# yinyunie/Pose2Room

Hardware: AMD Instinct MI355X
Metric: P2RNet train-step samples/sec (T=1024,J=53,bs=32) (higher is better)
Workload: dtype f32; 1 GPU; P2RNet full train step, bs=32/GPU, T=1024, J=53, seeds=512, proposals=128 (BASELINE configs[2]); input=P2RNet_dataloader over SyntheticPoseDataset, global_batch=32, frames=1024, parallelism=dp1

## Files before the change

### pose2room_amd/csrc/p2r_common.h

```cpp
#pragma once
#include <hip/hip_runtime.h>
#include <stdint.h>

#include "../../include/p2r_hip.h"

#pragma clang fp contract(off)

#define P2R_WAVE 64

#define P2R_LAUNCH_CHECK()                      \
  do {                                          \
    hipError_t e__ = hipGetLastError();         \
    if (e__ != hipSuccess) return (int)e__;     \
  } while (0)

static inline hipStream_t p2r_stream(void *s) { return (hipStream_t)s; }

static inline int p2r_ref_opt_n_threads(int work_size) {
  if (work_size <= 0) return 1;
  const int pow_2 = (int)(__builtin_log((double)work_size) / __builtin_log(2.0));
  int t = 1 << pow_2;
  if (t > 512) t = 512;
  if (t < 1) t = 1;
  return t;
}

static inline int p2r_cdiv(long long a, long long b) { return (int)((a + b - 1) / b); }

#define P2R_MAX_DEVICES 64
template <typename K>
static inline hipError_t p2r_allow_big_lds(K kernel, unsigned char (&done)[P2R_MAX_DEVICES], int bytes = 160 * 1024) {
  int dev = 0;
  hipError_t e = hipGetDevice(&dev);
  if (e != hipSuccess) return e;
  if (dev >= 0 && dev < P2R_MAX_DEVICES && done[dev]) return hipSuccess;
  e = hipFuncSetAttribute((const void *)kernel, hipFuncAttributeMaxDynamicSharedMemorySize, bytes);
  if (e == hipSuccess && dev >= 0 && dev < P2R_MAX_DEVICES) done[dev] = 1;
  return e;
}

template <auto KERNEL, typename... Args>
static inline int p2r_launch_big_lds(int blocks, int threads, size_t lds, void *stream, Args... args) {
  static unsigned char lds_ok[P2R_MAX_DEVICES];
  hipError_t e = p2r_allow_big_lds(KERNEL, lds_ok);
  if (e != hipSuccess) return (int)e;
  hipLaunchKernelGGL(KERNEL, dim3(blocks), dim3(threads), lds, p2r_stream(stream), args...);
  P2R_LAUNCH_CHECK();
  return P2R_OK;
}

__device__ __forceinline__ float p2r_sqdist(float ax, float ay, float az,
                                            float bx, float by, float bz) {
  const float dx = ax - bx, dy = ay - by, dz = az - bz;
  return dx * dx + dy * dy + dz * dz;
}

__device__ __forceinline__ float p2r_row16_sum(float v) {
  v += __int_as_float(__builtin_amdgcn_update_dpp(0, __float_as_int(v), 0xB1, 0xf, 0xf, false));
  v += __int_as_float(__builtin_amdgcn_update_dpp(0, __float_as_int(v), 0x4E, 0xf, 0xf, false));
  v += __int_as_float(__builtin_amdgcn_update_dpp(0, __float_as_int(v), 0x141, 0xf, 0xf, false));
  v += __int_as_float(__builtin_amdgcn_update_dpp(0, __float_as_int(v), 0x140, 0xf, 0xf, false));
  return v;
}
```

### pose2room_amd/csrc/pw_layers.hip

```cpp
#include "pw_mma.h"

namespace {

constexpr int PW_COLS = 64;
constexpr int PW_KMAX = 560;

struct PwJobs { p2r_pw_job j[P2R_PW_MAX_JOBS]; };

__global__ __launch_bounds__(256) void pw_gemm_kernel(PwJobs jobs, int L, int colblocks) {
  extern __shared__ float tile[];
  const p2r_pw_job &J = jobs.j[blockIdx.x / colblocks];
  const int cb = blockIdx.x % colblocks;
  const int col0 = cb * PW_COLS;
  const int b = col0 / L, l0 = col0 - b * L;
  const int tid = threadIdx.x, lane = tid & 63, wave = tid >> 6;
  const int g = lane >> 4, r = lane & 15;
  const int K = J.k, kpad = (K + 15) & ~15, rows = J.rows;

  if (!J.x_nlc) {
    const int c4 = tid & 15;
    const size_t base = (size_t)b * J.x_ctot * L + l0 + 4 * c4;
    for (int row = tid >> 4; row < kpad; row += 16) {
      float4 v = make_float4(0.f, 0.f, 0.f, 0.f);
      if (row < K) {
        v = *reinterpret_cast<const float4 *>(J.x + base + (size_t)row * L);
        if (J.tr_mode == 1) {
          const float s = J.tr[row], t = J.tr[J.tr_ld + row];
          v.x = fmaxf(v.x * s + t, 0.f); v.y = fmaxf(v.y * s + t, 0.f);
          v.z = fmaxf(v.z * s + t, 0.f); v.w = fmaxf(v.w * s + t, 0.f);
        } else if (J.tr_mode == 2) {
          const float4 z = *reinterpret_cast<const float4 *>(J.x2 + base + (size_t)row * L);
          const float a = J.tr[row], bq = J.tr[J.tr_ld + row], c = J.tr[2 * J.tr_ld + row];
          v.x = a * v.x + bq * z.x + c; v.y = a * v.y + bq * z.y + c;
          v.z = a * v.z + bq * z.z + c; v.w = a * v.w + bq * z.w + c;
        }
      }
      *reinterpret_cast<float4 *>(tile + row * PW_RS + 4 * c4) = v;
    }
  } else if ((K & 3) != 0 || (J.x_ctot & 3) != 0) {
    const int col = tid & 63;
    const size_t base = ((size_t)b * L + l0 + col) * J.x_ctot;
    for (int row = tid >> 6; row < kpad; row += 4) {
      float v = 0.f;
      if (row < K) {
        v = J.x[base + row];
        if (J.tr_mode == 1) v = fmaxf(v * J.tr[row] + J.tr[J.tr_ld + row], 0.f);
        else if (J.tr_mode == 2) v = J.tr[row] * v + J.tr[J.tr_ld + row] * J.x2[base + row] + J.tr[2 * J.tr_ld + row];
      }
      tile[row * PW_RS + col] = v;
    }
  } else {
    const int col = tid & 63;
    const size_t base = ((size_t)b * L + l0 + col) * J.x_ctot;
    for (int c4 = tid >> 6; c4 < (kpad >> 2); c4 += 4) {
      const int row = 4 * c4;
      float v[4] = {0.f, 0.f, 0.f, 0.f};
      if (row < K) {
        const float4 u = *reinterpret_cast<const float4 *>(J.x + base + row);
        v[0] = u.x; v[1] = u.y; v[2] = u.z; v[3] = u.w;
        if (J.tr_mode == 1) {
#pragma unroll
          for (int e = 0; e < 4; ++e) v[e] = fmaxf(v[e] * J.tr[row + e] + J.tr[J.tr_ld + row + e], 0.f);
        } else if (J.tr_mode == 2) {
          const float4 z4 = *reinterpret_cast<const float4 *>(J.x2 + base + row);
          const float z[4] = {z4.x, z4.y, z4.z, z4.w};
#pragma unroll
          for (int e = 0; e < 4; ++e)
            v[e] = J.tr[row + e] * v[e] + J.tr[J.tr_ld + row + e] * z[e] + J.tr[2 * J.tr_ld + row + e];
        }
      }
#pragma unroll
      for (int e = 0; e < 4; ++e) tile[(row + e) * PW_RS + col] = v[e];
    }
  }
  __syncthreads();

  const int mtiles = (rows + 15) >> 4;
  const int per = (mtiles + 3) >> 2;
  const int lo = wave * per, hi = min(lo + per, mtiles);
  const int nch = kpad >> 4;
  const bool nlc_vec = J.out_nlc && (rows & 3) == 0 && (J.out_ctot & 3) == 0 && (((size_t)J.out) & 15) == 0;
  for (int mt0 = lo; mt0 < hi; mt0 += 4) {
    const int nmt = min(4, hi - mt0);
    floatx4v acc[4][4];
#pragma unroll
    for (int m = 0; m < 4; ++m)
#pragma unroll
      for (int n = 0; n < 4; ++n) acc[m][n] = floatx4v{0.f, 0.f, 0.f, 0.f};
    int rowm[4];
#pragma unroll
    for (int m = 0; m < 4; ++m) rowm[m] = min(16 * (mt0 + m) + r, rows - 1);
    if (J.w_t) pw_product<true>(J.w, tile, K, rows, nch, nmt, rowm, g, r, acc);
    else pw_product<false>(J.w, tile, K, rows, nch, nmt, rowm, g, r, acc);

#pragma unroll
    for (int m = 0; m < 4; ++m) {
      if (m >= nmt) continue;
      const int row0 = 16 * (mt0 + m) + 4 * g;
      float v[4][4];
#pragma unroll
      for (int q = 0; q < 4; ++q) {
        const int row = row0 + q;
        const bool ok = row < rows;
        if (J.epilogue == 0) {
          const float bb = (J.bias && ok) ? J.bias[row] : 0.f;
#pragma unroll
          for (int n = 0; n < 4; ++n) v[q][n] = acc[m][n][q] + bb;
          if (J.stats) {
            float s = (v[q][0] + v[q][1]) + (v[q][2] + v[q][3]);
            s = p2r_row16_sum(s);
            const float mean = s * (1.f / 64.f);
            float d2 = 0.f;
#pragma unroll
            for (int n = 0; n < 4; ++n) { const float d = v[q][n] - mean; d2 += d * d; }
            d2 = p2r_row16_sum(d2);
            if (r == 0 && ok) {
              float *e = J.stats + ((size_t)cb * rows + row) * 3;
              e[0] = 64.f; e[1] = mean; e[2] = d2;
            }
          }
        } else {
          float sc = 0.f, sh = 0.f, mean = 0.f, invstd = 0.f;
          if (ok) {
            mean = J.mfin[row]; invstd = J.mfin[J.mfin_ld + row];
            sc = J.mfin[2 * J.mfin_ld + row]; sh = J.mfin[3 * J.mfin_ld + row];
          }
          float s1 = 0.f, s2 = 0.f;
#pragma unroll
          for (int n = 0; n < 4; ++n) {
            float z = 0.f;
            if (ok) z = J.mz[((size_t)b * J.mz_ctot + row) * L + l0 + 16 * n + r];
            const float gv = (z * sc + sh > 0.f) ? acc[m][n][q] : 0.f;
            v[q][n] = gv;
            s1 += gv;
            s2 += gv * ((z - mean) * invstd);
          }
          if (J.stats) {
            s1 = p2r_row16_sum(s1);
            s2 = p2r_row16_sum(s2);
            if (r == 0 && ok) {
              float *e = J.stats + ((size_t)cb * rows + row) * 2;
              e[0] = s1; e[1] = s2;
            }
          }
        }
      }
      if (!J.out_nlc) {
#pragma unroll
        for (int q = 0; q < 4; ++q)
          if (row0 + q < rows) {
            float *o = J.out + ((size_t)b * J.out_ctot + row0 + q) * L + l0 + r;
#pragma unroll
            for (int n = 0; n < 4; ++n) o[16 * n] = v[q][n];
          }
      } else {
#pragma unroll
        for (int n = 0; n < 4; ++n) {
          float *o = J.out + ((size_t)b * L + l0 + 16 * n + r) * J.out_ctot + row0;
          if (nlc_vec) {
            if (row0 < rows) *reinterpret_cast<float4 *>(o) = make_float4(v[0][n], v[1][n], v[2][n], v[3][n]);
          } else {
#pragma unroll
            for (int q = 0; q < 4; ++q)
              if (row0 + q < rows) o[q] = v[q][n];
          }
        }
      }
    }
  }
}

struct PwWJobs { p2r_pw_wjob j[P2R_PW_MAX_JOBS]; int blk0[P2R_PW_MAX_JOBS + 1]; };
constexpr int PWW_RS = 68;

__device__ __forceinline__ void pww_fetch(const float *__restrict__ p, int ctot, int nlc, int L, int b, int l0, int row_lo,
                                          int nrows, int tid, float4 (&v)[4]) {
#pragma unroll
  for (int i = 0; i < 4; ++i) {
    v[i] = make_float4(0.f, 0.f, 0.f, 0.f);
    if (!nlc) {
      const int row = row_lo + (tid >> 4) + 16 * i;
      if (row < nrows) v[i] = *reinterpret_cast<const float4 *>(p + ((size_t)b * ctot + row) * L + l0 + 4 * (tid & 15));
    } else {
      const int row = row_lo + 4 * ((tid >> 6) + 4 * i);
      const float *q = p + ((size_t)b * L + l0 + (tid & 63)) * ctot;
      if (((nrows | ctot) & 3) == 0) {
        if (row < nrows) v[i] = *reinterpret_cast<const float4 *>(q + row);
      } else {
        if (row + 0 < nrows) v[i].x = q[row + 0];
        if (row + 1 < nrows) v[i].y = q[row + 1];
        if (row + 2 < nrows) v[i].z = q[row + 2];
        if (row + 3 < nrows) v[i].w = q[row + 3];
      }
    }
  }
}

__global__ __launch_bounds__(256) void pw_wgrad_kernel(PwWJobs jobs, int L, int chunks) {
  __shared__ float as[64 * PWW_RS], bs[64 * PWW_RS];
  int ji = 0;
#pragma unroll
  for (int i = 1; i < P2R_PW_MAX_JOBS; ++i)
    if ((int)blockIdx.x >= jobs.blk0[i]) ji = i;
  const p2r_pw_wjob &J = jobs.j[ji];
  const int local = blockIdx.x - jobs.blk0[ji];
  const int rows = J.rows, K = J.k;
  const int tiles_m = (rows + 63) >> 6, tiles_n = (K + 63) >> 6;
  const int sp = local / (tiles_m * tiles_n), t = local % (tiles_m * tiles_n);
  const int tm = t / tiles_n, tn = t % tiles_n;
  const int cps = (chunks + J.split - 1) / J.split;
  const int c_lo = sp * cps, c_hi = min(c_lo + cps, chunks);
  const int tid = threadIdx.x, lane = tid & 63, wave = tid >> 6;
  const int g = lane >> 4, r = lane & 15;
  const int row_a = 64 * tm, row_b = 64 * tn;

  floatx4v acc[4];
#pragma unroll
  for (int mt = 0; mt < 4; ++mt) acc[mt] = floatx4v{0.f, 0.f, 0.f, 0.f};
  float bsum = 0.f;
  const bool want_b = J.db_part != nullptr && tn == 0;

  float4 ra[4], ra2[4], rb[4];
#pragma unroll
  for (int i = 0; i < 4; ++i) ra2[i] = make_float4(0.f, 0.f, 0.f, 0.f);
  if (c_lo < c_hi) {
    const int col0 = c_lo * 64, b = col0 / L, l0 = col0 - b * L;
    pww_fetch(J.x, J.x_ctot, J.x_nlc, L, b, l0, row_a, rows, tid, ra);
    if (J.tr_mode == 2) pww_fetch(J.x2, J.x_ctot, J.x_nlc, L, b, l0, row_a, rows, tid, ra2);
    pww_fetch(J.y, J.y_ctot, J.y_nlc, L, b, l0, row_b, K, tid, rb);
  }
  for (int c = c_lo; c < c_hi; ++c) {
    __syncthreads();
#pragma unroll
    for (int i = 0; i < 4; ++i) {
      const float va[4] = {ra[i].x, ra[i].y, ra[i].z, ra[i].w};
      const float vz[4] = {ra2[i].x, ra2[i].y, ra2[i].z, ra2[i].w};
      const float vb[4] = {rb[i].x, rb[i].y, rb[i].z, rb[i].w};
      if (!J.x_nlc) {
        const int lr = (tid >> 4) + 16 * i, row = row_a + lr;
        float o[4] = {0.f, 0.f, 0.f, 0.f};
        if (row < rows) {
          if (J.tr_mode == 2) {
            const float a = J.tr[row], bq = J.tr[J.tr_ld + row], cc = J.tr[2 * J.tr_ld + row];
#pragma unroll
            for (int e = 0; e < 4; ++e) o[e] = a * va[e] + bq * vz[e] + cc;
          } else {
#pragma unroll
            for (int e = 0; e < 4; ++e) o[e] = va[e];
          }
        }
        *reinterpret_cast<float4 *>(as + lr * PWW_RS + 4 * (tid & 15)) = make_float4(o[0], o[1], o[2], o[3]);
      } else {
#pragma unroll
        for (int e = 0; e < 4; ++e) {
          const int lr = 4 * ((tid >> 6) + 4 * i) + e, row = row_a + lr;
          float v = 0.f;
          if (row < rows) v = J.tr_mode == 2 ? J.tr[row] * va[e] + J.tr[J.tr_ld + row] * vz[e] + J.tr[2 * J.tr_ld + row] : va[e];
          as[lr * PWW_RS + (tid & 63)] = v;
        }
      }
      if (!J.y_nlc) {
        const int lr = (tid >> 4) + 16 * i, row = row_b + lr;
        float o[4] = {0.f, 0.f, 0.f, 0.f};
        if (row < K) {
          if (J.ytr) {
            const float sc = J.ytr[row], sh = J.ytr[J.ytr_ld + row];
#pragma unroll
            for (int e = 0; e < 4; ++e) o[e] = fmaxf(vb[e] * sc + sh, 0.f);
          } else {
#pragma unroll
            for (int e = 0; e < 4; ++e) o[e] = vb[e];
          }
        }
        *reinterpret_cast<float4 *>(bs + lr * PWW_RS + 4 * (tid & 15)) = make_float4(o[0], o[1], o[2], o[3]);
      } else {
#pragma unroll
        for (int e = 0; e < 4; ++e) {
          const int lr = 4 * ((tid >> 6) + 4 * i) + e, row = row_b + lr;
          float v = 0.f;
          if (row < K) v = J.ytr ? fmaxf(vb[e] * J.ytr[row] + J.ytr[J.ytr_ld + row], 0.f) : vb[e];
          bs[lr * PWW_RS + (tid & 63)] = v;
        }
      }
    }
    __syncthreads();
    if (c + 1 < c_hi) {
      const int col0 = (c + 1) * 64, b = col0 / L, l0 = col0 - b * L;
      pww_fetch(J.x, J.x_ctot, J.x_nlc, L, b, l0, row_a, rows, tid, ra);
      if (J.tr_mode == 2) pww_fetch(J.x2, J.x_ctot, J.x_nlc, L, b, l0, row_a, rows, tid, ra2);
      pww_fetch(J.y, J.y_ctot, J.y_nlc, L, b, l0, row_b, K, tid, rb);
    }
#pragma unroll 4
    for (int k = 0; k < 64; k += 4) {
      const float bv = bs[(16 * wave + r) * PWW_RS + k + g];
#pragma unroll
      for (int mt = 0; mt < 4; ++mt)
        acc[mt] = __builtin_amdgcn_mfma_f32_16x16x4f32(as[(16 * mt + r) * PWW_RS + k + g], bv, acc[mt], 0, 0, 0);
    }
    if (want_b) {
      const float *rowp = as + (tid >> 2) * PWW_RS + 16 * (tid & 3);
      float s = 0.f;
#pragma unroll
      for (int i = 0; i < 16; ++i) s += rowp[i];
      bsum += s;
    }
  }
  float *outp = J.dw_part + (size_t)sp * rows * K;
#pragma unroll
  for (int mt = 0; mt < 4; ++mt)
#pragma unroll
    for (int q = 0; q < 4; ++q) {
      const int row = row_a + 16 * mt + 4 * g + q, col = row_b + 16 * wave + r;
      if (row < rows && col < K) outp[(size_t)row * K + col] = acc[mt][q];
    }
  if (want_b) {
    bsum += __shfl_xor(bsum, 1);
    bsum += __shfl_xor(bsum, 2);
    const int row = row_a + (tid >> 2);
    if ((tid & 3) == 0 && row < rows) J.db_part[(size_t)sp * rows + row] = bsum;
  }
}

struct PwBnJobs { p2r_pw_bnjob j[P2R_PW_MAX_JOBS]; int ch0[P2R_PW_MAX_JOBS + 1]; };
struct PwBnbJobs { p2r_pw_bnbjob j[P2R_PW_MAX_JOBS]; int ch0[P2R_PW_MAX_JOBS + 1]; };

__device__ __forceinline__ double wave_sum(double v) {
#pragma unroll
  for (int off = 32; off >= 1; off >>= 1) v += __shfl_xor(v, off);
  return v;
}

__global__ __launch_bounds__(64) void pw_bn_finalize_kernel(PwBnJobs jobs) {
  int ji = 0;
#pragma unroll
  for (int i = 1; i < P2R_PW_MAX_JOBS; ++i)
    if ((int)blockIdx.x >= jobs.ch0[i]) ji = i;
  const p2r_pw_bnjob &J = jobs.j[ji];
  const int c = blockIdx.x - jobs.ch0[ji];
  const int lane = threadIdx.x;
  double mean, var, count = 0.0;
  if (J.part) {
    double n = 0.0, s = 0.0;
    for (int p = lane; p < J.P; p += 64) {
      const float *e = J.part + ((size_t)p * J.C + c) * 3;
      n += (double)e[0]; s += (double)e[0] * (double)e[1];
    }
    n = wave_sum(n); s = wave_sum(s);
    mean = s / n;
    double m2 = 0.0;
    for (int p = lane; p < J.P; p += 64) {
      const float *e = J.part + ((size_t)p * J.C + c) * 3;
      const double d = (double)e[1] - mean;
      m2 += (double)e[2] + (double)e[0] * d * d;
    }
    m2 = wave_sum(m2);
    var = m2 / n;
    if (var < 0.0) var = 0.0;
    count = n;
  } else {
    mean = (double)J.running_mean[c];
    var = (double)J.running_var[c];
  }
  if (lane == 0) {
    const float mean_f = (float)mean, invstd_f = (float)(1.0 / sqrt(var + J.eps));
    const float scale = J.gamma[c] * invstd_f;
    J.fin[c] = mean_f;
    J.fin[J.fin_ld + c] = invstd_f;
    J.fin[2 * J.fin_ld + c] = scale;
    J.fin[3 * J.fin_ld + c] = J.beta[c] - mean_f * scale;
    if (J.part && J.momentum >= 0.0) {
      const float mom = (float)J.momentum;
      const double unbiased = var * (count / (count - 1.0 > 1.0 ? count - 1.0 : 1.0));
      J.running_mean[c] = J.running_mean[c] * (1.f - mom) + mom * mean_f;
      J.running_var[c] = J.running_var[c] * (1.f - mom) + mom * (float)unbiased;
      if (c == 0 && J.num_batches_tracked) *J.num_batches_tracked += 1;
    }
  }
}

__global__ __launch_bounds__(64) void pw_bn_bwd_finalize_kernel(PwBnbJobs jobs) {
  int ji = 0;
#pragma unroll
  for (int i = 1; i < P2R_PW_MAX_JOBS; ++i)
    if ((int)blockIdx.x >= jobs.ch0[i]) ji = i;
  const p2r_pw_bnbjob &J = jobs.j[ji];
  const int c = blockIdx.x - jobs.ch0[ji];
  const int lane = threadIdx.x;
  double s = 0.0, q = 0.0;
  for (int p = lane; p < J.P; p += 64) {
    const float *e = J.part + ((size_t)p * J.C + c) * 2;
    s += (double)e[0]; q += (double)e[1];
  }
  s = wave_sum(s); q = wave_sum(q);
  if (lane == 0) {
    if (J.dbeta) J.dbeta[c] = (float)s;
    if (J.dgamma) J.dgamma[c] = (float)q;
    const float mean = J.fin[c], invstd = J.fin[J.fin_ld + c], scale = J.fin[2 * J.fin_ld + c];
    if (J.train) {
      const float m1 = (float)(s / J.M), m2 = (float)(q / J.M);
      J.coef[c] = scale;
      J.coef[J.coef_ld + c] = -scale * invstd * m2;
      J.coef[2 * J.coef_ld + c] = -scale * m1 + scale * invstd * m2 * mean;
    } else {
      J.coef[c] = scale;
      J.coef[J.coef_ld + c] = 0.f;
      J.coef[2 * J.coef_ld + c] = 0.f;
    }
  }
}

struct PwRJobs { p2r_pw_rjob j[P2R_PW_MAX_RJOBS]; int blk0[P2R_PW_MAX_RJOBS + 1]; };

__global__ __launch_bounds__(256) void pw_reduce_kernel(PwRJobs jobs, int njobs) {
  int ji = 0;
  for (int i = 1; i < njobs; ++i)
    if ((int)blockIdx.x >= jobs.blk0[i]) ji = i;
  const p2r_pw_rjob &J = jobs.j[ji];
  const int i = (blockIdx.x - jobs.blk0[ji]) * 256 + threadIdx.x;
  if (i >= J.M) return;
  float a0 = 0.f, a1 = 0.f, a2 = 0.f, a3 = 0.f;
  int p = 0;
  for (; p + 4 <= J.P; p += 4) {
    a0 += J.in[(size_t)(p + 0) * J.M + i];
    a1 += J.in[(size_t)(p + 1) * J.M + i];
    a2 += J.in[(size_t)(p + 2) * J.M + i];
    a3 += J.in[(size_t)(p + 3) * J.M + i];
  }
  for (; p < J.P; ++p) a0 += J.in[(size_t)p * J.M + i];
  J.out[i] = (a0 + a1) + (a2 + a3);
}

constexpr int MIX_DMAX = 4;
struct MixHeads { p2r_mix_head h[P2R_MIX_MAX_HEADS]; };

template <typename T>
__device__ __forceinline__ void mix_forward_body(const p2r_mix_head &H, int cols, int G, int L, int ctot, double *red) {
  const int tid = threadIdx.x, c = tid & 15, s = tid >> 4;
  const int col = blockIdx.x * 16 + c;
  const int D = H.D;
  const T *mu = (const T *)H.mu, *eps = (const T *)H.eps;
  T acc[MIX_DMAX];
#pragma unroll
  for (int d = 0; d < MIX_DMAX; ++d) acc[d] = (T)0;
  if (col < cols) {
    const int b = col / L, l = col - b * L;
    for (int gi = s; gi < G; gi += 16) {
      const float lg = H.logit[((size_t)b * ctot + gi) * L + l];
      const float p = 1.f / (1.f + expf(-lg));
      if (H.pi) H.pi[((size_t)b * G + gi) * L + l] = p;
#pragma unroll
      for (int d = 0; d < MIX_DMAX; ++d) {
        if (d < D) {
          T comp = mu[gi * D + d];
          if (eps) comp = eps[((size_t)col * G + gi) * D + d] * (T)expf(H.log_sigma[gi * D + d]) + comp;
          acc[d] += comp * (T)p;
        }
      }
    }
  }
#pragma unroll
  for (int d = 0; d < MIX_DMAX; ++d) red[(d * 16 + s) * 16 + c] = (double)acc[d];
  __syncthreads();
  if (tid < 16 * D) {
    const int d = tid >> 4, cc = tid & 15;
    T tot = (T)0;
    for (int i = 0; i < 16; ++i) tot += (T)red[(d * 16 + i) * 16 + cc];
    const int ocol = blockIdx.x * 16 + cc;
    if (ocol < cols) ((T *)H.pred)[(size_t)ocol * D + d] = tot;
  }
}

__global__ __launch_bounds__(256) void mdn_mix_forward_kernel(MixHeads heads, int cols, int G, int L, int ctot) {
  __shared__ double red[MIX_DMAX * 16 * 16];
  const p2r_mix_head &H = heads.h[blockIdx.y];
  if (H.f64) mix_forward_body<double>(H, cols, G, L, ctot, red);
  else mix_forward_body<float>(H, cols, G, L, ctot, red);
}

template <typename T>
__device__ __forceinline__ void mix_backward_body(const p2r_mix_head &H, int cols, int G, int L, int ctot, int dctot,
                                                  double (*red)[4]) {
  const int gi = blockIdx.x, tid = threadIdx.x;
  const int D = H.D;
  const T *mu = (const T *)H.mu, *eps = (const T *)H.eps, *dpred = (const T *)H.dpred;
  T muv[MIX_DMAX];
  float sig[MIX_DMAX];
#pragma unroll
  for (int d = 0; d < MIX_DMAX; ++d) {
    muv[d] = d < D ? mu[gi * D + d] : (T)0;
    sig[d] = d < D ? expf(H.log_sigma[gi * D + d]) : 0.f;
  }
  T smu[MIX_DMAX], ssg[MIX_DMAX];
#pragma unroll
  for (int d = 0; d < MIX_DMAX; ++d) { smu[d] = (T)0; ssg[d] = (T)0; }
  for (int col = tid; col < cols; col += 256) {
    const int b = col / L, l = col - b * L;
    const float lg = H.logit[((size_t)b * ctot + gi) * L + l];
    const float p = 1.f / (1.f + expf(-lg));
    T t = (T)0;
#pragma unroll
    for (int d = 0; d < MIX_DMAX; ++d) {
      if (d < D) {
        const T dp = dpred[(size_t)col * D + d];
        const T e = eps ? eps[((size_t)col * G + gi) * D + d] : (T)0;
        const T comp = e * (T)sig[d] + muv[d];
        t += dp * comp;
        const T dsamp = dp * (T)p;
        smu[d] += dsamp;
        ssg[d] += dsamp * e;
      }
    }
    H.dlogit[((size_t)b * dctot + gi) * L + l] = (float)t * (p * (1.f - p));
  }
#pragma unroll
  for (int d = 0; d < MIX_DMAX; ++d) {
    double a = (double)smu[d], c = (double)ssg[d];
    a = wave_sum(a); c = wave_sum(c);
    if ((tid & 63) == 0) { red[d][tid >> 6] = a; red[MIX_DMAX + d][tid >> 6] = c; }
  }
  __syncthreads();
  if (tid < D) {
    const double a = (red[tid][0] + red[tid][1]) + (red[tid][2] + red[tid][3]);
    const double c = (red[MIX_DMAX + tid][0] + red[MIX_DMAX + tid][1]) + (red[MIX_DMAX + tid][2] + red[MIX_DMAX + tid][3]);
    ((T *)H.dmu)[gi * D + tid] = (T)a;
    H.dlog_sigma[gi * D + tid] = (float)((T)c) * sig[tid];
  }
}

__global__ __launch_bounds__(256) void mdn_mix_backward_kernel(MixHeads heads, int cols, int G, int L, int ctot, int dctot) {
  __shared__ double red[2 * MIX_DMAX][4];
  const p2r_mix_head &H = heads.h[blockIdx.y];
  if (H.f64) mix_backward_body<double>(H, cols, G, L, ctot, dctot, red);
  else mix_backward_body<float>(H, cols, G, L, ctot, dctot, red);
}

}

extern "C" int p2r_pw_gemm(int njobs, const p2r_pw_job *jobs, int B, int L, void *stream) {
  if (njobs < 1 || njobs > P2R_PW_MAX_JOBS || B < 0 || L <= 0 || L % PW_COLS != 0 || !jobs) return P2R_EINVAL;
  if (B == 0) return P2R_OK;
  PwJobs pj;
  int kmax = 0;
  for (int i = 0; i < njobs; ++i) {
    const p2r_pw_job &j = jobs[i];
    const int kpad = (j.k + 15) & ~15;
    if (j.k <= 0 || j.rows <= 0 || kpad > PW_KMAX || !j.x || !j.w || !j.out) return P2R_EINVAL;
    if (!j.w_t && (j.k % 16 != 0 || (((size_t)j.w) & 15) != 0)) return P2R_EINVAL;
    if ((((size_t)j.x) & 15) != 0 || (j.tr_mode == 2 && (!j.x2 || (((size_t)j.x2) & 15) != 0))) return P2R_EINVAL;
    if (j.tr_mode != 0 && !j.tr) return P2R_EINVAL;
    if (j.epilogue == 1 && (!j.mz || !j.mfin)) return P2R_EINVAL;
    if (j.epilogue != 0 && j.epilogue != 1) return P2R_EINVAL;
    pj.j[i] = j;
    if (kpad > kmax) kmax = kpad;
  }
  const int colblocks = (int)((long long)B * L / PW_COLS);
  const int lds = kmax * PW_RS * (int)sizeof(float);
  static unsigned char lds_ok[P2R_MAX_DEVICES];
  hipError_t e = p2r_allow_big_lds(pw_gemm_kernel, lds_ok, PW_KMAX * PW_RS * (int)sizeof(float));
  if (e != hipSuccess) return (int)e;
  hipLaunchKernelGGL(pw_gemm_kernel, dim3((unsigned)(njobs * colblocks)), dim3(256), lds, p2r_stream(stream), pj, L,
                     colblocks);
  P2R_LAUNCH_CHECK();
  return P2R_OK;
}

extern "C" int p2r_pw_wgrad(int njobs, const p2r_pw_wjob *jobs, int B, int L, void *stream) {
  if (njobs < 1 || njobs > P2R_PW_MAX_JOBS || B < 0 || L <= 0 || L % 64 != 0 || !jobs) return P2R_EINVAL;
  if (B == 0) return P2R_OK;
  PwWJobs pj;
  int total = 0;
  for (int i = 0; i < P2R_PW_MAX_JOBS + 1; ++i) pj.blk0[i] = 0x7fffffff;
  for (int i = 0; i < njobs; ++i) {
    const p2r_pw_wjob &j = jobs[i];
    if (j.rows <= 0 || j.k <= 0 || j.split < 1 || !j.x || !j.y || !j.dw_part) return P2R_EINVAL;
    if (j.tr_mode != 0 && j.tr_mode != 2) return P2R_EINVAL;
    if (j.tr_mode == 2 && (!j.x2 || !j.tr)) return P2R_EINVAL;
    if ((((size_t)j.x) & 15) != 0 || (((size_t)j.y) & 15) != 0 || (j.x2 && (((size_t)j.x2) & 15) != 0)) return P2R_EINVAL;
    pj.j[i] = j;
    pj.blk0[i] = total;
    total += ((j.rows + 63) / 64) * ((j.k + 63) / 64) * j.split;
  }
  pj.blk0[0] = 0;
  const int chunks = (int)((long long)B * L / 64);
  hipLaunchKernelGGL(pw_wgrad_kernel, dim3((unsigned)total), dim3(256), 0, p2r_stream(stream), pj, L, chunks);
  P2R_LAUNCH_CHECK();
  return P2R_OK;
}

extern "C" int p2r_pw_bn_finalize(int njobs, const p2r_pw_bnjob *jobs, void *stream) {
  if (njobs < 1 || njobs > P2R_PW_MAX_JOBS || !jobs) return P2R_EINVAL;
  PwBnJobs pj;
  int total = 0;
  for (int i = 0; i < P2R_PW_MAX_JOBS + 1; ++i) pj.ch0[i] = 0x7fffffff;
  for (int i = 0; i < njobs; ++i) {
    const p2r_pw_bnjob &j = jobs[i];
    if (j.C <= 0 || !j.gamma || !j.beta || !j.fin || (j.part && j.P <= 0)) return P2R_EINVAL;
    if (!j.part && (!j.running_mean || !j.running_var)) return P2R_EINVAL;
    if (j.part && j.momentum >= 0.0 && (!j.running_mean || !j.running_var)) return P2R_EINVAL;
    pj.j[i] = j;
    pj.ch0[i] = total;
    total += j.C;
  }
  pj.ch0[0] = 0;
  hipLaunchKernelGGL(pw_bn_finalize_kernel, dim3((unsigned)total), dim3(64), 0, p2r_stream(stream), pj);
  P2R_LAUNCH_CHECK();
  return P2R_OK;
}

extern "C" int p2r_pw_bn_bwd_finalize(int njobs, const p2r_pw_bnbjob *jobs, void *stream) {
  if (njobs < 1 || njobs > P2R_PW_MAX_JOBS || !jobs) return P2R_EINVAL;
  PwBnbJobs pj;
  int total = 0;
  for (int i = 0; i < P2R_PW_MAX_JOBS + 1; ++i) pj.ch0[i] = 0x7fffffff;
  for (int i = 0; i < njobs; ++i) {
    const p2r_pw_bnbjob &j = jobs[i];
    if (j.C <= 0 || j.P <= 0 || !j.part || !j.fin || !j.coef || j.M <= 0.0) return P2R_EINVAL;
    pj.j[i] = j;
    pj.ch0[i] = total;
    total += j.C;
  }
  pj.ch0[0] = 0;
  hipLaunchKernelGGL(pw_bn_bwd_finalize_kernel, dim3((unsigned)total), dim3(64), 0, p2r_stream(stream), pj);
  P2R_LAUNCH_CHECK();
  return P2R_OK;
}

extern "C" int p2r_pw_reduce(int njobs, const p2r_pw_rjob *jobs, void *stream) {
  if (njobs < 1 || njobs > P2R_PW_MAX_RJOBS || !jobs) return P2R_EINVAL;
  PwRJobs pj;
  int total = 0;
  for (int i = 0; i < P2R_PW_MAX_RJOBS + 1; ++i) pj.blk0[i] = 0x7fffffff;
  for (int i = 0; i < njobs; ++i) {
    const p2r_pw_rjob &j = jobs[i];
    if (j.P <= 0 || j.M <= 0 || !j.in || !j.out) return P2R_EINVAL;
    pj.j[i] = j;
    pj.blk0[i] = total;
    total += (j.M + 255) / 256;
  }
  pj.blk0[0] = 0;
  hipLaunchKernelGGL(pw_reduce_kernel, dim3((unsigned)total), dim3(256), 0, p2r_stream(stream), pj, njobs);
  P2R_LAUNCH_CHECK();
  return P2R_OK;
}

extern "C" int p2r_mdn_mix_forward(int nheads, const p2r_mix_head *heads, int B, int G, int L, int logit_ctot,
                                   void *stream) {
  if (nheads < 1 || nheads > P2R_MIX_MAX_HEADS || !heads || B < 0 || G <= 0 || L <= 0) return P2R_EINVAL;
  if (B == 0) return P2R_OK;
  MixHeads mh;
  for (int i = 0; i < nheads; ++i) {
    const p2r_mix_head &h = heads[i];
    if (h.D <= 0 || h.D > MIX_DMAX || !h.logit || !h.mu || !h.pred || (h.eps && !h.log_sigma)) return P2R_EINVAL;
    mh.h[i] = h;
  }
  const int cols = B * L;
  hipLaunchKernelGGL(mdn_mix_forward_kernel, dim3((unsigned)p2r_cdiv(cols, 16), (unsigned)nheads), dim3(256), 0,
                     p2r_stream(stream), mh, cols, G, L, logit_ctot);
  P2R_LAUNCH_CHECK();
  return P2R_OK;
}

extern "C" int p2r_mdn_mix_backward(int nheads, const p2r_mix_head *heads, int B, int G, int L, int logit_ctot,
                                    int dlogit_ctot, void *stream) {
  if (nheads < 1 || nheads > P2R_MIX_MAX_HEADS || !heads || B <= 0 || G <= 0 || L <= 0) return P2R_EINVAL;
  MixHeads mh;
  for (int i = 0; i < nheads; ++i) {
    const p2r_mix_head &h = heads[i];
    if (h.D <= 0 || h.D > MIX_DMAX || !h.logit || !h.mu || !h.log_sigma || !h.dpred || !h.dlogit || !h.dmu ||
        !h.dlog_sigma)
      return P2R_EINVAL;
    mh.h[i] = h;
  }
  hipLaunchKernelGGL(mdn_mix_backward_kernel, dim3((unsigned)G, (unsigned)nheads), dim3(256), 0, p2r_stream(stream), mh,
                     B * L, G, L, logit_ctot, dlogit_ctot);
  P2R_LAUNCH_CHECK();
  return P2R_OK;
}
```

### pose2room_amd/csrc/sa_votes.hip

```cpp
#include "pw_mma.h"

namespace {

constexpr int SA_C = 256;
constexpr int SA_S = 16;
constexpr int SA_BALLS = 4;
constexpr int SA_COLS = SA_BALLS * SA_S;
constexpr int SA_RS = PW_RS;

__device__ __forceinline__ void sa_layer(const float *__restrict__ W, const float *__restrict__ act,
                                         int wave, int g, int r, floatx4v (&acc)[4][4]) {
#pragma unroll
  for (int m = 0; m < 4; ++m)
#pragma unroll
    for (int n = 0; n < 4; ++n) acc[m][n] = floatx4v{0.f, 0.f, 0.f, 0.f};
  int rowm[4];
#pragma unroll
  for (int m = 0; m < 4; ++m) rowm[m] = 64 * wave + 16 * m + r;
  pw_product<false>(W, act, SA_C, SA_C, SA_C / 16, 4, rowm, g, r, acc);
}

template <bool TRAIN>
__global__ __launch_bounds__(256, 2) void sa_votes_kernel(int n, int m, float radius2, const float *__restrict__ xyz,
                                                       const float *__restrict__ new_xyz,
                                                       const float *__restrict__ features,
                                                       const float *__restrict__ w1, const float *__restrict__ b1,
                                                       const float *__restrict__ w2, const float *__restrict__ b2,
                                                       int *__restrict__ idx, float *__restrict__ out,
                                                       float *__restrict__ G, float *__restrict__ H,
                                                       unsigned char *__restrict__ amax) {
  extern __shared__ float lds[];
  float *gs = lds;
  float *hs = lds;
  __shared__ int s_idx[SA_BALLS][SA_S];

  const int tid = threadIdx.x, lane = tid & 63, wave = tid >> 6;
  const int g = lane >> 4, r = lane & 15;
  const int groups = (m + SA_BALLS - 1) / SA_BALLS;
  const int batch = blockIdx.x / groups;
  const int j0 = (blockIdx.x % groups) * SA_BALLS;
  const float *pts = xyz + (size_t)batch * n * 3;
  const float *feat = features + (size_t)batch * SA_C * n;

  {
    const int j = j0 + wave;
    int cnt = 0, first = 0;
    if (j < m) {
      const float cx = new_xyz[((size_t)batch * m + j) * 3 + 0];
      const float cy = new_xyz[((size_t)batch * m + j) * 3 + 1];
      const float cz = new_xyz[((size_t)batch * m + j) * 3 + 2];
      const unsigned long long lt_mask = (lane == 0) ? 0ull : (~0ull >> (64 - lane));
      for (int k0 = 0; k0 < n && cnt < SA_S; k0 += 64) {
        const int k = k0 + lane;
        bool hit = false;
        if (k < n) hit = p2r_sqdist(cx, cy, cz, pts[k * 3 + 0], pts[k * 3 + 1], pts[k * 3 + 2]) < radius2;
        const unsigned long long mask = __ballot(hit);
        if (mask != 0ull) {
          if (cnt == 0) first = k0 + (int)__builtin_ctzll(mask);
          const int slot = cnt + (int)__builtin_popcountll(mask & lt_mask);
          if (hit && slot < SA_S) s_idx[wave][slot] = k;
          cnt += (int)__builtin_popcountll(mask);
        }
      }
    }
    const int filled = min(cnt, SA_S);
    if (lane >= filled && lane < SA_S) s_idx[wave][lane] = cnt > 0 ? first : 0;
  }
  __syncthreads();
  if (tid < SA_COLS) {
    const int j = j0 + (tid >> 4);
    if (j < m) idx[((size_t)batch * m + j) * SA_S + (tid & 15)] = s_idx[tid >> 4][tid & 15];
  }

  {
    const int col = tid & 63;
    const int src = s_idx[col >> 4][col & 15];
    const int jc = j0 + (col >> 4);
    for (int c = tid >> 6; c < SA_C; c += 4) {
      const float v = feat[(size_t)c * n + src];
      gs[c * SA_RS + col] = v;
      if (TRAIN && jc < m) G[(((size_t)batch * SA_C + c) * m + jc) * SA_S + (col & 15)] = v;
    }
  }
  __syncthreads();

  floatx4v acc[4][4];
  sa_layer(w1, gs, wave, g, r, acc);
  __syncthreads();
#pragma unroll
  for (int mt = 0; mt < 4; ++mt)
#pragma unroll
    for (int q = 0; q < 4; ++q) {
      const int row = 64 * wave + 16 * mt + 4 * g + q;
      const float bb = b1[row];
#pragma unroll
      for (int nt = 0; nt < 4; ++nt) {
        const float h = fmaxf(acc[mt][nt][q] + bb, 0.f);
        hs[row * SA_RS + 16 * nt + r] = h;
        if (TRAIN && j0 + nt < m) H[(((size_t)batch * SA_C + row) * m + j0 + nt) * SA_S + r] = h;
      }
    }
  __syncthreads();
  sa_layer(w2, hs, wave, g, r, acc);
#pragma unroll
  for (int mt = 0; mt < 4; ++mt)
#pragma unroll
    for (int q = 0; q < 4; ++q) {
      const int row = 64 * wave + 16 * mt + 4 * g + q;
      const float bb = b2[row];
#pragma unroll
      for (int nt = 0; nt < 4; ++nt) {
        float v = fmaxf(acc[mt][nt][q] + bb, 0.f);
        int am = r;
#pragma unroll
        for (int off = 8; off >= 1; off >>= 1) {
          const float ov = __shfl_xor(v, off, 16);
          const int oa = __shfl_xor(am, off, 16);
          if (ov > v || (ov == v && oa < am)) { v = ov; am = oa; }
        }
        const int j = j0 + nt;
        if (r == 0 && j < m) {
          out[((size_t)batch * SA_C + row) * m + j] = v;
          if (TRAIN) amax[((size_t)batch * SA_C + row) * m + j] = (unsigned char)am;
        }
      }
    }
}

__global__ __launch_bounds__(256, 2) void sa_votes_backward_kernel(int m, const float *__restrict__ dout,
                                                                const float *__restrict__ out,
                                                                const unsigned char *__restrict__ amax,
                                                                const float *__restrict__ H,
                                                                const float *__restrict__ w2t,
                                                                const float *__restrict__ w1t,
                                                                float *__restrict__ dZ2, float *__restrict__ dZ1,
                                                                float *__restrict__ dG) {
  extern __shared__ float lds[];
  float *zs = lds;
  float *ys = lds;
  const int tid = threadIdx.x, lane = tid & 63, wave = tid >> 6;
  const int g = lane >> 4, r = lane & 15;
  const int groups = (m + SA_BALLS - 1) / SA_BALLS;
  const int batch = blockIdx.x / groups;
  const int j0 = (blockIdx.x % groups) * SA_BALLS;

  {
    const int col = tid & 63, ball = col >> 4, smp = col & 15;
    const int j = j0 + ball;
    for (int c = tid >> 6; c < SA_C; c += 4) {
      float v = 0.f;
      if (j < m) {
        const size_t o = ((size_t)batch * SA_C + c) * m + j;
        if ((int)amax[o] == smp && out[o] > 0.f) v = dout[o];
        dZ2[o * SA_S + smp] = v;
      }
      zs[c * SA_RS + col] = v;
    }
  }
  __syncthreads();
  floatx4v acc[4][4];
  sa_layer(w2t, zs, wave, g, r, acc);
  __syncthreads();
#pragma unroll
  for (int mt = 0; mt < 4; ++mt)
#pragma unroll
    for (int q = 0; q < 4; ++q) {
      const int row = 64 * wave + 16 * mt + 4 * g + q;
#pragma unroll
      for (int nt = 0; nt < 4; ++nt) {
        float v = 0.f;
        if (j0 + nt < m) {
          const size_t o = (((size_t)batch * SA_C + row) * m + j0 + nt) * SA_S + r;
          v = H[o] > 0.f ? acc[mt][nt][q] : 0.f;
          dZ1[o] = v;
        }
        ys[row * SA_RS + 16 * nt + r] = v;
      }
    }
  __syncthreads();
  sa_layer(w1t, ys, wave, g, r, acc);
#pragma unroll
  for (int mt = 0; mt < 4; ++mt)
#pragma unroll
    for (int q = 0; q < 4; ++q) {
      const int row = 64 * wave + 16 * mt + 4 * g + q;
#pragma unroll
      for (int nt = 0; nt < 4; ++nt)
        if (j0 + nt < m) dG[(((size_t)batch * SA_C + row) * m + j0 + nt) * SA_S + r] = acc[mt][nt][q];
    }
}

constexpr int GN_CH = 64;
constexpr int GN_RS = GN_CH + 1;
__global__ __launch_bounds__(256) void gemm_nt_kernel(int nb, int L, int split, const float *__restrict__ A,
                                                      const float *__restrict__ B, float *__restrict__ partial) {
  __shared__ float as[64 * GN_RS], bs[64 * GN_RS];
  const int tid = threadIdx.x, lane = tid & 63, wave = tid >> 6;
  const int g = lane >> 4, r = lane & 15;
  const int tile = blockIdx.x % 16, part = blockIdx.x / 16;
  const int m0 = (tile >> 2) * 64, n0 = (tile & 3) * 64;
  const long long total = (long long)nb * L;
  const long long per = ((total + split - 1) / split + GN_CH - 1) / GN_CH * GN_CH;
  const long long lo = part * per, hi = lo + per < total ? lo + per : total;
  floatx4v acc[4];
#pragma unroll
  for (int mt = 0; mt < 4; ++mt) acc[mt] = floatx4v{0.f, 0.f, 0.f, 0.f};
  for (long long c0 = lo; c0 < hi; c0 += GN_CH) {
    __syncthreads();
    if (L % GN_CH == 0 && c0 + GN_CH <= hi) {
      const long long bidx = c0 / L, l = c0 - bidx * L;
      for (int e = tid; e < 64 * (GN_CH / 4); e += 256) {
        const int row = e >> 4, c4 = e & 15;
        const float4 va = *reinterpret_cast<const float4 *>(A + ((size_t)bidx * 256 + m0 + row) * L + l + 4 * c4);
        const float4 vb = *reinterpret_cast<const float4 *>(B + ((size_t)bidx * 256 + n0 + row) * L + l + 4 * c4);
        float *pa = as + row * GN_RS + 4 * c4, *pb = bs + row * GN_RS + 4 * c4;
        pa[0] = va.x; pa[1] = va.y; pa[2] = va.z; pa[3] = va.w;
        pb[0] = vb.x; pb[1] = vb.y; pb[2] = vb.z; pb[3] = vb.w;
      }
    } else {
      for (int e = tid; e < 64 * GN_CH; e += 256) {
        const int row = e >> 6, cc = e & 63;
        const long long col = c0 + cc;
        float va = 0.f, vb = 0.f;
        if (col < hi) {
          const long long bidx = col / L, l = col - bidx * L;
          va = A[((size_t)bidx * 256 + m0 + row) * L + l];
          vb = B[((size_t)bidx * 256 + n0 + row) * L + l];
        }
        as[row * GN_RS + cc] = va;
        bs[row * GN_RS + cc] = vb;
      }
    }
    __syncthreads();
#pragma unroll 4
    for (int k = 0; k < GN_CH; k += 4) {
      const float b = bs[(16 * wave + r) * GN_RS + k + g];
#pragma unroll
      for (int mt = 0; mt < 4; ++mt)
        acc[mt] = __builtin_amdgcn_mfma_f32_16x16x4f32(as[(16 * mt + r) * GN_RS + k + g], b, acc[mt], 0, 0, 0);
    }
  }
  float *outp = partial + (size_t)part * 256 * 256;
#pragma unroll
  for (int mt = 0; mt < 4; ++mt)
#pragma unroll
    for (int q = 0; q < 4; ++q) outp[(size_t)(m0 + 16 * mt + 4 * g + q) * 256 + n0 + 16 * wave + r] = acc[mt][q];
}

}

extern "C" int p2r_sa_votes_forward(int b, int n, int m, int nsample, float radius, int C0, int C1, int C2,
                                    const float *xyz, const float *new_xyz, const float *features,
                                    const float *w1, const float *b1, const float *w2, const float *b2,
                                    int *idx, float *out, float *G, float *H, unsigned char *amax, void *stream) {
  if (b < 0 || n <= 0 || m < 0) return P2R_EINVAL;
  const bool train = G != nullptr;
  if (train && (!H || !amax)) return P2R_EINVAL;
  if (nsample != SA_S || C0 != SA_C || C1 != SA_C || C2 != SA_C) return P2R_EINVAL;
  if (b == 0 || m == 0) return P2R_OK;
  const int groups = (m + SA_BALLS - 1) / SA_BALLS;
  const size_t lds = (size_t)SA_C * SA_RS * sizeof(float);
  auto kern = train ? sa_votes_kernel<true> : sa_votes_kernel<false>;
  static unsigned char lds_ok[2][P2R_MAX_DEVICES];
  hipError_t e = p2r_allow_big_lds(kern, lds_ok[train ? 1 : 0], (int)lds);
  if (e != hipSuccess) return (int)e;
  hipLaunchKernelGGL(kern, dim3((unsigned)(b * groups)), dim3(256), lds, p2r_stream(stream), n, m,
                     radius * radius, xyz, new_xyz, features, w1, b1, w2, b2, idx, out, G, H, amax);
  P2R_LAUNCH_CHECK();
  return P2R_OK;
}

extern "C" int p2r_sa_votes_backward(int b, int m, int nsample, int C, const float *dout, const float *out,
                                     const unsigned char *amax, const float *H, const float *w2t, const float *w1t,
                                     float *dZ2, float *dZ1, float *dG, void *stream) {
  if (b < 0 || m < 0 || nsample != SA_S || C != SA_C) return P2R_EINVAL;
  if (b == 0 || m == 0) return P2R_OK;
  const int groups = (m + SA_BALLS - 1) / SA_BALLS;
  const size_t lds = (size_t)SA_C * SA_RS * sizeof(float);
  static unsigned char lds_ok[P2R_MAX_DEVICES];
  hipError_t e = p2r_allow_big_lds(sa_votes_backward_kernel, lds_ok, (int)lds);
  if (e != hipSuccess) return (int)e;
  hipLaunchKernelGGL(sa_votes_backward_kernel, dim3((unsigned)(b * groups)), dim3(256), lds, p2r_stream(stream), m,
                     dout, out, amax, H, w2t, w1t, dZ2, dZ1, dG);
  P2R_LAUNCH_CHECK();
  return P2R_OK;
}

extern "C" int p2r_gemm_nt_256(int nb, int L, int split, const float *A, const float *B, float *partial, void *stream) {
  if (nb < 0 || L <= 0 || split < 1 || split > 1024) return P2R_EINVAL;
  if (nb == 0) return P2R_OK;
  hipLaunchKernelGGL(gemm_nt_kernel, dim3(16 * split), dim3(256), 0, p2r_stream(stream), nb, L, split, A, B, partial);
  P2R_LAUNCH_CHECK();
  return P2R_OK;
}
```

### pose2room_amd/csrc/seed_ops.hip

```cpp
#include "p2r_common.h"

namespace {

__global__ __launch_bounds__(256) void gather_frames_kernel(int C, int T, int J, int S, const float *__restrict__ x,
                                                            const long long *__restrict__ inds, float *__restrict__ out) {
  const int b = blockIdx.x / S;
  const long long t = inds[blockIdx.x];
  const int n = C * J;
  float *o = out + (size_t)blockIdx.x * n;
  if (t < 0 || t >= T) {
    for (int e = threadIdx.x; e < n; e += 256) o[e] = 0.f;
    return;
  }
  const float *xb = x + ((size_t)b * C * T + t) * J;
  for (int e = threadIdx.x; e < n; e += 256) {
    const int c = e / J, j = e - c * J;
    o[e] = xb[(size_t)c * T * J + j];
  }
}

constexpr int GF_TT = 8;
constexpr int GF_MAXHIT = 16;

__global__ __launch_bounds__(256) void gather_frames_grad_kernel(int C, int T, int J, int S,
                                                                 const float *__restrict__ dout,
                                                                 const long long *__restrict__ inds,
                                                                 float *__restrict__ dx) {
  __shared__ int hits[GF_TT][GF_MAXHIT];
  __shared__ int nhit[GF_TT];
  const int chunks = (T + GF_TT - 1) / GF_TT;
  const int b = blockIdx.x / chunks, t0 = (blockIdx.x - b * chunks) * GF_TT;
  const int tid = threadIdx.x, lane = tid & 63, wave = tid >> 6;
  for (int f = 2 * wave; f < 2 * wave + 2; ++f) {
    const long long t = t0 + f;
    int cnt = 0;
    const unsigned long long lt = lane == 0 ? 0ull : (~0ull >> (64 - lane));
    for (int s0 = 0; s0 < S; s0 += 64) {
      const int s = s0 + lane;
      const bool hit = s < S && inds[(size_t)b * S + s] == t;
      const unsigned long long m = __ballot(hit);
      const int slot = cnt + (int)__builtin_popcountll(m & lt);
      if (hit && slot < GF_MAXHIT) hits[f][slot] = s;
      cnt += (int)__builtin_popcountll(m);
    }
    if (lane == 0) nhit[f] = cnt;
  }
  __syncthreads();
  const int n = C * J, run = GF_TT * J;
  for (int e = tid; e < run; e += 256) {
    const int f = e / J, j = e - f * J;
    if (t0 + f >= T) continue;
    const int cnt = nhit[f];
    float *xb = dx + ((size_t)b * C * T + t0) * J + e;
    if (cnt <= 2) {
      const float *r0 = dout + ((size_t)b * S + (cnt > 0 ? hits[f][0] : 0)) * n + j;
      const float *r1 = dout + ((size_t)b * S + (cnt > 1 ? hits[f][1] : 0)) * n + j;
      int c = 0;
      for (; c + 8 <= C; c += 8) {
        float v[8];
#pragma unroll
        for (int u = 0; u < 8; ++u) {
          v[u] = cnt > 0 ? r0[(c + u) * J] : 0.f;
          if (cnt > 1) v[u] += r1[(c + u) * J];
        }
#pragma unroll
        for (int u = 0; u < 8; ++u) xb[(size_t)(c + u) * T * J] = v[u];
      }
      for (; c < C; ++c) {
        float v = cnt > 0 ? r0[c * J] : 0.f;
        if (cnt > 1) v += r1[c * J];
        xb[(size_t)c * T * J] = v;
      }
      continue;
    }
    for (int c = 0; c < C; ++c) {
      float acc = 0.f;
      if (cnt <= GF_MAXHIT) {
        for (int i = 0; i < cnt; ++i) acc += dout[((size_t)b * S + hits[f][i]) * n + c * J + j];
      } else {
        for (int s = 0; s < S; ++s)
          if (inds[(size_t)b * S + s] == (long long)(t0 + f)) acc += dout[((size_t)b * S + s) * n + c * J + j];
      }
      xb[(size_t)c * T * J] = acc;
    }
  }
}

__global__ __launch_bounds__(256) void rowsum_short_kernel(long long rows, int V, float scale, const float *__restrict__ x,
                                                           float *__restrict__ out) {
  extern __shared__ float tile[];
  const long long r0 = (long long)blockIdx.x * 256;
  const int nr = (int)(rows - r0 < 256 ? rows - r0 : 256);
  const int n = nr * V, Vp = V | 1;
  const float *src = x + r0 * V;
  for (int i = threadIdx.x; i < n; i += 256) {
    const int r = i / V, v = i - r * V;
    tile[r * Vp + v] = src[i];
  }
  __syncthreads();
  if ((int)threadIdx.x < nr) {
    const float *p = tile + threadIdx.x * Vp;
    float a0 = 0.f, a1 = 0.f;
    int v = 0;
    for (; v + 2 <= V; v += 2) { a0 += p[v]; a1 += p[v + 1]; }
    if (v < V) a0 += p[v];
    out[r0 + threadIdx.x] = (a0 + a1) * scale;
  }
}

constexpr int VF_C = 256, VF_COLS = 64, VF_RS = VF_COLS + 1;

__global__ __launch_bounds__(256) void vote_finish_kernel(int S, const float *__restrict__ net,
                                                          const float *__restrict__ seed_features,
                                                          const float *__restrict__ hip, float *__restrict__ vote_xyz,
                                                          float *__restrict__ feat_ncl, float *__restrict__ inv_norm) {
  extern __shared__ float tile[];
  const int tid = threadIdx.x, lane = tid & 63, wave = tid >> 6;
  const size_t col0 = (size_t)blockIdx.x * VF_COLS;
  const int b = (int)(col0 / S), s0 = (int)(col0 - (size_t)b * S);
  for (int i = 0; i < 16; ++i) {
    const int cl = 16 * wave + i;
    const size_t col = col0 + cl;
    const float *nr = net + col * (3 + VF_C);
    const float *sr = seed_features + col * VF_C;
    float f[4];
#pragma unroll
    for (int e = 0; e < 4; ++e) f[e] = sr[lane + 64 * e] + nr[3 + lane + 64 * e];
    float ss = (f[0] * f[0] + f[1] * f[1]) + (f[2] * f[2] + f[3] * f[3]);
#pragma unroll
    for (int off = 32; off >= 1; off >>= 1) ss += __shfl_xor(ss, off, 64);
    const float inv = 1.f / sqrtf(ss);
#pragma unroll
    for (int e = 0; e < 4; ++e) tile[(lane + 64 * e) * VF_RS + cl] = f[e] * inv;
    if (lane < 3) vote_xyz[col * 3 + lane] = hip[col * 3 + lane] + nr[lane];
    if (lane == 3) inv_norm[col] = inv;
  }
  __syncthreads();
  float *ob = feat_ncl + (size_t)b * VF_C * S + s0;
  for (int c = wave; c < VF_C; c += 4) ob[(size_t)c * S + lane] = tile[c * VF_RS + lane];
}

__global__ __launch_bounds__(256) void vote_finish_grad_kernel(int S, const float *__restrict__ d_xyz,
                                                               const float *__restrict__ d_feat,
                                                               const float *__restrict__ feat,
                                                               const float *__restrict__ inv_norm,
                                                               float *__restrict__ d_net, float *__restrict__ d_sf) {
  extern __shared__ float tile[];
  float *dy = tile, *y = tile + VF_C * VF_RS;
  const int tid = threadIdx.x, lane = tid & 63, wave = tid >> 6;
  const size_t col0 = (size_t)blockIdx.x * VF_COLS;
  const int b = (int)(col0 / S), s0 = (int)(col0 - (size_t)b * S);
  const float *gb = d_feat + (size_t)b * VF_C * S + s0, *yb = feat + (size_t)b * VF_C * S + s0;
  for (int c = wave; c < VF_C; c += 4) {
    dy[c * VF_RS + lane] = d_feat ? gb[(size_t)c * S + lane] : 0.f;
    y[c * VF_RS + lane] = yb[(size_t)c * S + lane];
  }
  __syncthreads();
  for (int i = 0; i < 16; ++i) {
    const int cl = 16 * wave + i;
    const size_t col = col0 + cl;
    float g[4], v[4];
#pragma unroll
    for (int e = 0; e < 4; ++e) { g[e] = dy[(lane + 64 * e) * VF_RS + cl]; v[e] = y[(lane + 64 * e) * VF_RS + cl]; }
    float dot = (g[0] * v[0] + g[1] * v[1]) + (g[2] * v[2] + g[3] * v[3]);
#pragma unroll
    for (int off = 32; off >= 1; off >>= 1) dot += __shfl_xor(dot, off, 64);
    const float inv = inv_norm[col];
    float df[4];
#pragma unroll
    for (int e = 0; e < 4; ++e) df[e] = inv * (g[e] - v[e] * dot);
    float *nr = d_net + col * (3 + VF_C);
#pragma unroll
    for (int e = 0; e < 4; ++e) {
      nr[3 + lane + 64 * e] = df[e];
      d_sf[col * VF_C + lane + 64 * e] = df[e];
    }
    if (lane < 3) nr[lane] = d_xyz ? d_xyz[col * 3 + lane] : 0.f;
  }
}

__global__ __launch_bounds__(256) void nearest_prefix_kernel(int T, int S, const float *__restrict__ cum,
                                                             const float *__restrict__ target,
                                                             long long *__restrict__ inds) {
  extern __shared__ float row[];
  const int b = blockIdx.y;
  for (int t = threadIdx.x; t < T; t += 256) row[t] = cum[(size_t)b * T + t];
  __syncthreads();
  const int s = blockIdx.x * 256 + threadIdx.x;
  if (s >= S) return;
  const float tg = target[(size_t)b * S + s];
  float best = fabsf(row[0] - tg);
  int arg = 0;
  for (int t = 1; t < T; ++t) {
    const float d = fabsf(row[t] - tg);
    if (d < best) { best = d; arg = t; }
  }
  inds[(size_t)b * S + s] = arg;
}

}

extern "C" int p2r_gather_frames(int b, int c, int t, int j, int s, const float *x, const long long *inds, float *out,
                                 void *stream) {
  if (b < 0 || c <= 0 || t <= 0 || j <= 0 || s < 0) return P2R_EINVAL;
  if (b == 0 || s == 0) return P2R_OK;
  hipLaunchKernelGGL(gather_frames_kernel, dim3((unsigned)(b * s)), dim3(256), 0, p2r_stream(stream), c, t, j, s, x, inds,
                     out);
  P2R_LAUNCH_CHECK();
  return P2R_OK;
}

extern "C" int p2r_gather_frames_grad(int b, int c, int t, int j, int s, const float *dout, const long long *inds,
                                      float *dx, void *stream) {
  if (b < 0 || c <= 0 || t <= 0 || j <= 0 || s < 0) return P2R_EINVAL;
  if (b == 0) return P2R_OK;
  hipLaunchKernelGGL(gather_frames_grad_kernel, dim3((unsigned)(b * ((t + GF_TT - 1) / GF_TT))), dim3(256), 0,
                     p2r_stream(stream), c, t, j, s, dout, inds, dx);
  P2R_LAUNCH_CHECK();
  return P2R_OK;
}

extern "C" int p2r_rowsum_short(long long rows, int v_len, float scale, const float *x, float *out, void *stream) {
  if (rows < 0 || v_len < 1 || v_len > 64) return P2R_EINVAL;
  if (rows == 0) return P2R_OK;
  const size_t lds = 256 * (size_t)(v_len | 1) * sizeof(float);
  hipLaunchKernelGGL(rowsum_short_kernel, dim3((unsigned)((rows + 255) / 256)), dim3(256), lds, p2r_stream(stream), rows,
                     v_len, scale, x, out);
  P2R_LAUNCH_CHECK();
  return P2R_OK;
}

extern "C" int p2r_vote_finish(int b, int s, int C, const float *net, const float *seed_features, const float *hip,
                               float *vote_xyz, float *feat_ncl, float *inv_norm, void *stream) {
  if (b < 0 || s <= 0 || s % VF_COLS != 0 || C != VF_C) return P2R_EINVAL;
  if (b == 0) return P2R_OK;
  const size_t lds = (size_t)VF_C * VF_RS * sizeof(float);
  static unsigned char lds_ok[P2R_MAX_DEVICES];
  hipError_t e = p2r_allow_big_lds(vote_finish_kernel, lds_ok, (int)lds);
  if (e != hipSuccess) return (int)e;
  hipLaunchKernelGGL(vote_finish_kernel, dim3((unsigned)((size_t)b * s / VF_COLS)), dim3(256), lds, p2r_stream(stream), s, net,
                     seed_features, hip, vote_xyz, feat_ncl, inv_norm);
  P2R_LAUNCH_CHECK();
  return P2R_OK;
}

extern "C" int p2r_vote_finish_grad(int b, int s, int C, const float *d_xyz, const float *d_feat, const float *feat_ncl,
                                    const float *inv_norm, float *d_net, float *d_sf, void *stream) {
  if (b < 0 || s <= 0 || s % VF_COLS != 0 || C != VF_C) return P2R_EINVAL;
  if (b == 0) return P2R_OK;
  const size_t lds = (size_t)2 * VF_C * VF_RS * sizeof(float);
  static unsigned char lds_ok[P2R_MAX_DEVICES];
  hipError_t e = p2r_allow_big_lds(vote_finish_grad_kernel, lds_ok, (int)lds);
  if (e != hipSuccess) return (int)e;
  hipLaunchKernelGGL(vote_finish_grad_kernel, dim3((unsigned)((size_t)b * s / VF_COLS)), dim3(256), lds, p2r_stream(stream),
                     s, d_xyz, d_feat, feat_ncl, inv_norm, d_net, d_sf);
  P2R_LAUNCH_CHECK();
  return P2R_OK;
}

extern "C" int p2r_nearest_prefix(int b, int t, int s, const float *cum, const float *target, long long *inds,
                                  void *stream) {
  if (b < 0 || t <= 0 || s < 0 || t > 40000) return P2R_EINVAL;
  if (b == 0 || s == 0) return P2R_OK;
  static unsigned char lds_ok[P2R_MAX_DEVICES];
  hipError_t e = p2r_allow_big_lds(nearest_prefix_kernel, lds_ok, 40000 * (int)sizeof(float));
  if (e != hipSuccess) return (int)e;
  hipLaunchKernelGGL(nearest_prefix_kernel, dim3((unsigned)((s + 255) / 256), (unsigned)b), dim3(256),
                     (size_t)t * sizeof(float), p2r_stream(stream), t, s, cum, target, inds);
  P2R_LAUNCH_CHECK();
  return P2R_OK;
}
```

### pose2room_amd/csrc/stgcn_tconv.hip

```cpp
#include "p2r_common.h"

namespace {

typedef float floatx4c __attribute__((ext_vector_type(4)));

constexpr int TC_C = 64;
constexpr int TC_NPO = 384;
constexpr int TC_THREADS = 512;
constexpr int TC_NT = 3;

template <int TAPS>
__global__ __launch_bounds__(TC_THREADS, 2) void tconv_fused_kernel(
    int n_seq, int T, int V, int F, int tiles_per_seq, int row_len, const float *__restrict__ x,
    const float *__restrict__ scale, const float *__restrict__ shift, const float *__restrict__ W,
    const float *__restrict__ bias, float *__restrict__ out, float *__restrict__ stats_partial) {
  extern __shared__ float hs[];
  constexpr int HALO = (TAPS - 1) / 2;
  constexpr int NCH = TAPS == 1 ? TC_NPO / 64 : 8;

  const int tid = threadIdx.x, lane = tid & 63, wave = __builtin_amdgcn_readfirstlane(tid >> 6);
  const int g = lane >> 4, r = lane & 15;
  const size_t row_stride = (size_t)T * V;
  const int rs = (int)row_stride;
  const int total_tiles = n_seq * tiles_per_seq;

  float pre[8][NCH];
  auto issue_loads = [&](int tile) __attribute__((always_inline)) {
    const int seq = tile / tiles_per_seq;
    const int t0 = (tile % tiles_per_seq) * F;
    const int frames = min(F, T - t0);
    const int col0 = (t0 - HALO) * V;
    const int bytes = 4 * min(rs, col0 + (frames + 2 * HALO) * V);
    const float *xg = x + (size_t)seq * TC_C * row_stride;
#pragma unroll
    for (int h = 0; h < 8; ++h) {
      const __amdgpu_buffer_rsrc_t rsrc = __builtin_amdgcn_make_buffer_rsrc(
          const_cast<float *>(xg + (size_t)(wave + 8 * h) * row_stride), 0, bytes, 0x00020000);
#pragma unroll
      for (int i = 0; i < NCH; ++i)
        pre[h][i] = __uint_as_float(__builtin_amdgcn_raw_buffer_load_b32(rsrc, 4 * lane + 4 * (col0 + 64 * i), 0, 0));
    }
  };

  float *rowstat = hs + TC_C * row_len;
  for (int e = tid; e < (TC_THREADS / 64) * 2 * TC_C; e += TC_THREADS) rowstat[e] = 0.f;

  int tile = blockIdx.x;
  if (tile < total_tiles) issue_loads(tile);
  for (; tile < total_tiles; tile += gridDim.x) {
    const int seq = tile / tiles_per_seq;
    const int t0 = (tile % tiles_per_seq) * F;
    const int frames = min(F, T - t0);
    const int ncols = frames * V;
    float *og = out + (size_t)seq * TC_C * row_stride + (size_t)t0 * V;

    bool in[NCH];
#pragma unroll
    for (int i = 0; i < NCH; ++i) {
      const int q = lane + 64 * i, gc = (t0 - HALO) * V + q;
      in[i] = q < (frames + 2 * HALO) * V && gc >= 0 && gc < rs;
    }
#pragma unroll
    for (int h = 0; h < 8; ++h) {
      const int c = wave + 8 * h;
      const float sc = scale ? scale[c] : 1.f, sh = scale ? shift[c] : 0.f;
#pragma unroll
      for (int i = 0; i < NCH; ++i) {
        const int q = lane + 64 * i;
        float v = pre[h][i];
        if (scale) v = fmaxf(fmaf(v, sc, sh), 0.f);
        v = in[i] ? v : 0.f;
        if (q < row_len) hs[c * row_len + q] = v;
      }
    }
    __syncthreads();
    if (tile + (int)gridDim.x < total_tiles) issue_loads(tile + gridDim.x);

    int colv[TC_NT], base[TC_NT];
    bool valid[TC_NT];
#pragma unroll
    for (int i = 0; i < TC_NT; ++i) {
      const int col = (wave * TC_NT + i) * 16 + r;
      colv[i] = col;
      valid[i] = col < ncols;
      base[i] = valid[i] ? col : 0;
    }
    floatx4c acc[TC_NT][4];
#pragma unroll
    for (int m = 0; m < 4; ++m)
#pragma unroll
      for (int q = 0; q < 4; ++q) {
        const float bv = bias ? bias[16 * m + 4 * g + q] : 0.f;
#pragma unroll
        for (int i = 0; i < TC_NT; ++i) acc[i][m][q] = bv;
      }

    const float *hg = hs + g * 16 * row_len;
#pragma unroll 1
    for (int ph = 0; ph < 2 * TAPS; ++ph) {
      const int p = ph >> 1, hf = ph & 1;
      float a[4][8];
#pragma unroll
      for (int m = 0; m < 4; ++m) {
        const float4 *wp = reinterpret_cast<const float4 *>(W + ((size_t)p * TC_C + 16 * m + r) * TC_C + 16 * g + 8 * hf);
#pragma unroll
        for (int q = 0; q < 2; ++q) {
          const float4 u = wp[q];
          a[m][4 * q + 0] = u.x; a[m][4 * q + 1] = u.y; a[m][4 * q + 2] = u.z; a[m][4 * q + 3] = u.w;
        }
      }
#pragma unroll
      for (int i = 0; i < TC_NT; ++i) {
        const float *hb = hg + base[i] + p * V + 8 * hf * row_len;
        float b[8];
#pragma unroll
        for (int s2 = 0; s2 < 8; ++s2) b[s2] = valid[i] ? hb[s2 * row_len] : 0.f;
#pragma unroll
        for (int s2 = 0; s2 < 8; ++s2)
#pragma unroll
          for (int m = 0; m < 4; ++m)
            acc[i][m] = __builtin_amdgcn_mfma_f32_16x16x4f32(a[m][s2], b[s2], acc[i][m], 0, 0, 0);
      }
    }

#pragma unroll
    for (int m = 0; m < 4; ++m)
#pragma unroll
      for (int q = 0; q < 4; ++q) {
        const int row = 16 * m + 4 * g + q;
        float s1 = 0.f, s2 = 0.f;
#pragma unroll
        for (int i = 0; i < TC_NT; ++i) {
          if (!valid[i]) continue;
          const float v = acc[i][m][q];
          og[(size_t)row * row_stride + colv[i]] = v;
          s1 += v;
          s2 = fmaf(v, v, s2);
        }
        if (stats_partial) {
          s1 = p2r_row16_sum(s1);
          s2 = p2r_row16_sum(s2);
          if (r == 0) {
            float *slot = rowstat + wave * 2 * TC_C + 2 * row;
            slot[0] += s1;
            slot[1] += s2;
          }
        }
      }
    __syncthreads();
  }
  __syncthreads();
  if (stats_partial && tid < 2 * TC_C) {
    float tot = 0.f;
#pragma unroll
    for (int w = 0; w < TC_THREADS / 64; ++w) tot += rowstat[w * 2 * TC_C + tid];
    stats_partial[(size_t)blockIdx.x * 2 * TC_C + tid] = tot;
  }
}

constexpr int TW_F = 4;
#define TW_WAVES 16
constexpr int TW_THREADS = 64 * TW_WAVES;
constexpr int TW_MT = 4 / (TW_WAVES / 4);

__host__ __device__ constexpr int tw_row(int cols) {
  int r = cols + 7;
  while (r % 32 != 2) ++r;
  return r;
}
template <int TAPS, int VS, int F = TW_F, bool DZ = false, bool XF = true, bool AMAX = false>
__global__ __launch_bounds__(TW_THREADS, TW_WAVES == 8 ? 2 : 1) void tconv_dw_kernel(
    int n_seq, int T, int V_, int row_d_, int row_h_, const float *__restrict__ x,
    const float *__restrict__ scale, const float *__restrict__ shift, const float *__restrict__ dout,
    float *__restrict__ dw_partial, float *__restrict__ dbias_partial, const float *__restrict__ dh = nullptr,
    const float *__restrict__ fin = nullptr, const float *__restrict__ m12 = nullptr, float *__restrict__ dz = nullptr,
    unsigned *__restrict__ amax = nullptr) {
  static_assert(!AMAX || DZ, "the range word belongs to dz");
  unsigned am = 0;
  constexpr int HALO = (TAPS - 1) / 2;
  constexpr int NH = VS > 0 ? ((F + 2 * HALO) * VS + 63) / 64 : (TAPS == 1 ? 4 : 6);
  const int V = VS > 0 ? VS : V_;
  const int row_d = VS > 0 ? tw_row(F * VS) : row_d_, row_h = VS > 0 ? tw_row((F + 2 * HALO) * VS) : row_h_;
  static_assert(!DZ || VS > 0, "the fused BatchNorm-backward form exists for the unrolled instances");
  constexpr int ZI0 = DZ ? (HALO * VS) / 64 : 0, ZI1 = DZ ? ((HALO + F) * VS - 1) / 64 : -1, NZ = ZI1 - ZI0 + 1;
  extern __shared__ float lds[];
  float *ds = lds;
  float *hs = lds + TC_C * row_d;

  const int tid = threadIdx.x, lane = tid & 63, wave = __builtin_amdgcn_readfirstlane(tid >> 6);
  const int g = lane >> 4, r = lane & 15;
  const int nt = wave & 3, mh = wave >> 2;
  const int tiles_per_seq = (T + F - 1) / F;
  const int total_tiles = n_seq * tiles_per_seq;
  const size_t row_stride = (size_t)T * V;

  for (int e = tid; e < TC_C * (row_d + row_h); e += TW_THREADS) lds[e] = 0.f;

  float bsum[TC_C / (TW_THREADS / 64)];
#pragma unroll
  for (int h = 0; h < TC_C / (TW_THREADS / 64); ++h) bsum[h] = 0.f;
  floatx4c acc[TAPS][TW_MT];
#pragma unroll
  for (int p = 0; p < TAPS; ++p)
#pragma unroll
    for (int m = 0; m < TW_MT; ++m) acc[p][m] = floatx4c{0.f, 0.f, 0.f, 0.f};

  constexpr int NR = TC_C / (TW_THREADS / 64);
  float ph_[NR][NH], pd_[NR][4], pz_[NR][NZ > 0 ? NZ : 1];
  constexpr int PER_ROW = NH + 4 + NZ, PIECES = NR * PER_ROW;
  const int rs = (int)row_stride;
  const int lane4 = lane * 4;
  size_t ld_off = 0;
  int ld_t0v = 0, ld_col0 = 0, ld_hcols = 0, ld_hbytes = 0, ld_dbytes = 0, ld_zbytes = 0;
  auto set_tile = [&](int tile, bool valid) __attribute__((always_inline)) {
    const int seq = tile / tiles_per_seq;
    const int t0 = (tile % tiles_per_seq) * F;
    const int frames = min(F, T - t0);
    ld_hcols = (frames + 2 * HALO) * V;
    ld_off = (size_t)seq * TC_C * row_stride;
    ld_t0v = t0 * V;
    ld_col0 = (t0 - HALO) * V;
    ld_hbytes = valid ? 4 * min(rs, ld_col0 + ld_hcols) : 0;
    ld_dbytes = valid ? 4 * frames * V : 0;
    ld_zbytes = valid ? 4 * (ld_t0v + frames * V) : 0;
  };
  auto issue_piece = [&](int j) __attribute__((always_inline)) {
    const int hh = j / PER_ROW, i = j % PER_ROW;
    const int c = wave + hh * (TW_THREADS / 64);
    const size_t row = ld_off + (size_t)c * row_stride;
    if (i < NH) {
      const __amdgpu_buffer_rsrc_t rsrc = __builtin_amdgcn_make_buffer_rsrc(const_cast<float *>(x + row), 0, ld_hbytes, 0x00020000);
      ph_[hh][i] = __uint_as_float(__builtin_amdgcn_raw_buffer_load_b32(rsrc, lane4 + 4 * (ld_col0 + 64 * i), 0, 0));
    } else if (i < NH + 4) {
      const __amdgpu_buffer_rsrc_t rsrc =
          __builtin_amdgcn_make_buffer_rsrc(const_cast<float *>(dout + row + ld_t0v), 0, ld_dbytes, 0x00020000);
      pd_[hh][i - NH] = __uint_as_float(__builtin_amdgcn_raw_buffer_load_b32(rsrc, lane4 + 256 * (i - NH), 0, 0));
    } else {
      const int iz = i - NH - 4;
      const __amdgpu_buffer_rsrc_t rsrc = __builtin_amdgcn_make_buffer_rsrc(const_cast<float *>(dh + row), 0, ld_zbytes, 0x00020000);
      pz_[hh][iz] = __uint_as_float(__builtin_amdgcn_raw_buffer_load_b32(rsrc, lane4 + 4 * (ld_col0 + 64 * (ZI0 + iz)), 0, 0));
    }
  };
  auto issue_loads = [&](int tile) __attribute__((always_inline)) {
    set_tile(tile, true);
#pragma unroll
    for (int hh = 0; hh < NR; ++hh)
#pragma unroll
      for (int i = 0; i < PER_ROW; ++i) issue_piece(hh * PER_ROW + i);
  };

  int tile = blockIdx.x;
  if (tile < total_tiles) issue_loads(tile);
  for (; tile < total_tiles; tile += gridDim.x) {
    __syncthreads();
    const bool interior = VS > 0 && ld_col0 >= 0 && ld_col0 + (F + 2 * HALO) * V <= rs;
    bool hin[NH];
#pragma unroll
    for (int i = 0; i < NH; ++i) {
      const int q = lane + 64 * i, gc = ld_col0 + q;
      hin[i] = interior ? q < (F + 2 * HALO) * V : (q < ld_hcols && gc >= 0 && gc < rs);
    }
#pragma unroll
    for (int hh = 0; hh < NR; ++hh) {
      const int c = wave + hh * (TW_THREADS / 64);
      const float sc = XF ? scale[c] : 1.f, sh = XF ? shift[c] : 0.f;
      bsum[hh] += (pd_[hh][0] + pd_[hh][1]) + (pd_[hh][2] + pd_[hh][3]);
      if constexpr (DZ) {
        const float mu = fin[c], is = fin[64 + c], kk = sc, a1 = m12[c], a2 = m12[64 + c];
        const __amdgpu_buffer_rsrc_t rsrc = __builtin_amdgcn_make_buffer_rsrc(
            dz + ld_off + (size_t)c * row_stride, 0, ld_zbytes, 0x00020000);
#pragma unroll
        for (int iz = 0; iz < NZ; ++iz) {
          const int i = ZI0 + iz;
          const float zv = ph_[hh][i];
          const float gq = fmaf(zv, sc, sh) > 0.f ? pz_[hh][iz] : 0.f;
          const float xh = (zv - mu) * is;
          const float o = kk * (gq - a1 - xh * a2);
          if (64 * i >= HALO * VS || lane + 64 * i >= HALO * VS) {
            __builtin_amdgcn_raw_buffer_store_b32(__float_as_uint(o), rsrc, lane4 + 4 * (ld_col0 + 64 * i), 0, 0);
            if (AMAX && (unsigned)(lane4 + 4 * (ld_col0 + 64 * i)) < (unsigned)ld_zbytes)
              am = max(am, __float_as_uint(o) & 0x7fffffffu);
          }
        }
      }
#pragma unroll
      for (int i = 0; i < NH; ++i) {
        const int q = lane + 64 * i;
        float v = ph_[hh][i];
        if (XF) v = fmaxf(fmaf(v, sc, sh), 0.f);
        if (!(VS > 0 && interior && 64 * (i + 1) <= (F + 2 * HALO) * VS)) v = hin[i] ? v : 0.f;
        if (q < row_h) hs[c * row_h + q] = v;
      }
#pragma unroll
      for (int i = 0; i < 4; ++i) {
        const int q = lane + 64 * i;
        if (q < row_d) ds[c * row_d + q] = pd_[hh][i];
      }
    }
    __syncthreads();
    const bool more = tile + (int)gridDim.x < total_tiles;
    if constexpr (VS > 0) {
      set_tile(more ? tile + gridDim.x : tile, more);
    } else {
      if (more) issue_loads(tile + gridDim.x);
    }

    const float *drow = ds + (16 * TW_MT * mh + r) * row_d + g;
    const float *hrow = hs + (16 * nt + r) * row_h + g;
    float a[TW_MT], b[TAPS];
#pragma unroll
    for (int m = 0; m < TW_MT; ++m) a[m] = drow[16 * m * row_d];
    if constexpr (VS > 0) {
      constexpr int STEPS = (F * VS + 3) / 4;
      constexpr int PPS = (PIECES + STEPS - 1) / STEPS;
#pragma unroll
      for (int p = 0; p < TAPS; ++p) b[p] = hrow[p * VS];
#pragma unroll
      for (int s = 0; s < STEPS; ++s) {
        float na[TW_MT], nb[TAPS];
#pragma unroll
        for (int k = 0; k < PPS; ++k)
          if (PPS * s + k < PIECES) issue_piece(PPS * s + k);
#pragma unroll
        for (int m = 0; m < TW_MT; ++m) na[m] = drow[16 * m * row_d + 4 * s + 4];
#pragma unroll
        for (int p = 0; p < TAPS; ++p) nb[p] = hrow[p * VS + 4 * s + 4];
        __builtin_amdgcn_sched_barrier(0);
#pragma unroll
        for (int p = 0; p < TAPS; ++p)
#pragma unroll
          for (int m = 0; m < TW_MT; ++m)
            acc[p][m] = __builtin_amdgcn_mfma_f32_16x16x4f32(a[m], b[p], acc[p][m], 0, 0, 0);
        __builtin_amdgcn_sched_barrier(0);
#pragma unroll
        for (int m = 0; m < TW_MT; ++m) a[m] = na[m];
#pragma unroll
        for (int p = 0; p < TAPS; ++p) b[p] = nb[p];
      }
    } else {
      const int steps = (F * V + 3) / 4;
#pragma unroll
      for (int p = 0; p < TAPS; ++p) b[p] = hrow[p * V];
      for (int s = 0; s < steps; ++s) {
        float na[TW_MT], nb[TAPS];
#pragma unroll
        for (int m = 0; m < TW_MT; ++m) na[m] = drow[16 * m * row_d + 4 * s + 4];
#pragma unroll
        for (int p = 0; p < TAPS; ++p) nb[p] = hrow[p * V + 4 * s + 4];
#pragma unroll
        for (int p = 0; p < TAPS; ++p)
#pragma unroll
          for (int m = 0; m < TW_MT; ++m)
            acc[p][m] = __builtin_amdgcn_mfma_f32_16x16x4f32(a[m], b[p], acc[p][m], 0, 0, 0);
#pragma unroll
        for (int m = 0; m < TW_MT; ++m) a[m] = na[m];
#pragma unroll
        for (int p = 0; p < TAPS; ++p) b[p] = nb[p];
      }
    }
  }
  if constexpr (AMAX) {
#pragma unroll
    for (int off = 32; off >= 1; off >>= 1) am = max(am, (unsigned)__shfl_xor((int)am, off, 64));
    if (lane == 0 && am != 0) atomicMax(amax, am);
  }
  if (dbias_partial) {
#pragma unroll
    for (int hh = 0; hh < TC_C / (TW_THREADS / 64); ++hh) {
      float v = bsum[hh];
#pragma unroll
      for (int off = 32; off >= 1; off >>= 1) v += __shfl_xor(v, off, 64);
      if (lane == 0) dbias_partial[(size_t)blockIdx.x * TC_C + wave + hh * (TW_THREADS / 64)] = v;
    }
  }
  float *outp = dw_partial + (size_t)blockIdx.x * TAPS * TC_C * TC_C;
#pragma unroll
  for (int p = 0; p < TAPS; ++p)
#pragma unroll
    for (int m = 0; m < TW_MT; ++m)
#pragma unroll
      for (int q = 0; q < 4; ++q)
        outp[((size_t)(16 * TW_MT * mh + 16 * m + 4 * g + q) * TC_C + 16 * nt + r) * TAPS + p] = acc[p][m][q];
}

}

template <int TAPS>
static int tconv_forward_launch(int N, int T, int V, const float *x, const float *scale, const float *shift,
                                const float *W, const float *bias, float *out, float *stats_partial,
                                int *n_partials, void *stream) {
  constexpr int HALO = (TAPS - 1) / 2;
  int F = TC_NPO / V;
  if (F < 1) return P2R_EINVAL;
  if (F > T) F = T;
  const int tiles_per_seq = p2r_cdiv(T, F);
  int row_len = (F + 2 * HALO) * V;
  if (row_len % 2 == 0) ++row_len;
  const size_t lds = (size_t)TC_C * row_len * sizeof(float) + (size_t)(TC_THREADS / 64) * 2 * TC_C * sizeof(float);
  if (lds > 160 * 1024 || row_len > 512) return P2R_EINVAL;
  if ((long long)T * V >= (1LL << 29)) return P2R_EINVAL;
  static unsigned char lds_ok[P2R_MAX_DEVICES];
  {
    hipError_t e = p2r_allow_big_lds(tconv_fused_kernel<TAPS>, lds_ok);
    if (e != hipSuccess) return (int)e;
  }
  const long long tiles = (long long)N * tiles_per_seq;
  if (tiles > 0x7fffffffLL) return P2R_EINVAL;
  const int blocks = (int)(tiles < 256 ? tiles : 256);
  if (n_partials) *n_partials = blocks;
  if (!out) return P2R_OK;
  hipLaunchKernelGGL(tconv_fused_kernel<TAPS>, dim3(blocks), dim3(TC_THREADS), lds, p2r_stream(stream), N, T, V,
                     F, tiles_per_seq, row_len, x, scale, shift, W, bias, out, stats_partial);
  P2R_LAUNCH_CHECK();
  return P2R_OK;
}

extern "C" int p2r_stgcn_tconv_forward(int N, int T, int V, int taps, const float *x, const float *scale,
                                       const float *shift, const float *W, const float *bias, float *out,
                                       float *stats_partial, int *n_partials, void *stream) {
  if (N < 0 || T <= 0 || V <= 0 || V > 128 || (taps != 1 && taps != 3)) return P2R_EINVAL;
  if (n_partials) *n_partials = 0;
  if (N == 0) return P2R_OK;
  return taps == 3 ? tconv_forward_launch<3>(N, T, V, x, scale, shift, W, bias, out, stats_partial, n_partials, stream)
                   : tconv_forward_launch<1>(N, T, V, x, scale, shift, W, bias, out, stats_partial, n_partials, stream);
}

template <int TAPS, int VS, int F = TW_F, bool DZ = false, bool AMAX = false>
static int tconv_dw_launch(int N, int T, int V, const float *x, const float *scale, const float *shift,
                           const float *dout, int n_blocks, float *dw_partial, float *dbias_partial,
                           void *stream, const float *dh = nullptr, const float *fin = nullptr, const float *m12 = nullptr,
                           float *dz = nullptr, unsigned *amax = nullptr) {
  constexpr int HALO = (TAPS - 1) / 2;
  const int row_d = tw_row(F * V), row_h = tw_row((F + 2 * HALO) * V);
  const size_t lds = (size_t)TC_C * (row_d + row_h) * sizeof(float);
  if (lds > 160 * 1024 || F * V > 256 || (F + 2 * HALO) * V > (TAPS == 1 ? 256 : 384)) return P2R_EINVAL;
  if ((long long)T * V >= (1LL << 29)) return P2R_EINVAL;
  static unsigned char lds_ok[2][P2R_MAX_DEVICES];
  if (scale || DZ) {
    hipError_t e = p2r_allow_big_lds(tconv_dw_kernel<TAPS, VS, F, DZ, true, AMAX>, lds_ok[0]);
    if (e != hipSuccess) return (int)e;
    hipLaunchKernelGGL((tconv_dw_kernel<TAPS, VS, F, DZ, true, AMAX>), dim3(n_blocks), dim3(TW_THREADS), lds,
                       p2r_stream(stream), N, T, V, row_d, row_h, x, scale, shift, dout, dw_partial, dbias_partial, dh, fin,
                       m12, dz, amax);
  } else {
    hipError_t e = p2r_allow_big_lds(tconv_dw_kernel<TAPS, VS, F, false, false>, lds_ok[1]);
    if (e != hipSuccess) return (int)e;
    hipLaunchKernelGGL((tconv_dw_kernel<TAPS, VS, F, false, false>), dim3(n_blocks), dim3(TW_THREADS), lds, p2r_stream(stream),
                       N, T, V, row_d, row_h, x, scale, shift, dout, dw_partial, dbias_partial, dh, fin, m12, dz);
  }
  P2R_LAUNCH_CHECK();
  return P2R_OK;
}

extern "C" int p2r_stgcn_tconv_weight_grad(int N, int T, int V, int taps, const float *x, const float *scale,
                                           const float *shift, const float *dout, int n_blocks,
                                           float *dw_partial, float *dbias_partial, void *stream) {
  if (N < 0 || T <= 0 || V <= 0 || V > 64 || n_blocks < 1 || (taps != 1 && taps != 3)) return P2R_EINVAL;
  if (N == 0) return P2R_OK;
  if (V == 20 && taps == 1)
    return tconv_dw_launch<1, 20, 12>(N, T, V, x, scale, shift, dout, n_blocks, dw_partial, dbias_partial, stream);
  if (V == 53)
    return taps == 3
               ? tconv_dw_launch<3, 53>(N, T, V, x, scale, shift, dout, n_blocks, dw_partial, dbias_partial, stream)
               : tconv_dw_launch<1, 53>(N, T, V, x, scale, shift, dout, n_blocks, dw_partial, dbias_partial, stream);
  return taps == 3 ? tconv_dw_launch<3, 0>(N, T, V, x, scale, shift, dout, n_blocks, dw_partial, dbias_partial, stream)
                   : tconv_dw_launch<1, 0>(N, T, V, x, scale, shift, dout, n_blocks, dw_partial, dbias_partial, stream);
}

extern "C" int p2r_stgcn_tconv_weight_grad_dz(int N, int T, int V, int taps, const float *x, const float *fin,
                                              const float *dout, const float *dh, const float *m12, float *dz,
                                              int n_blocks, float *dw_partial, float *dbias_partial, void *stream) {
  if (N < 0 || T <= 0 || V != 53 || taps != 3 || n_blocks < 1 || !fin || !dh || !m12 || !dz) return P2R_EINVAL;
  if (N == 0) return P2R_OK;
  return tconv_dw_launch<3, 53, TW_F, true>(N, T, V, x, fin + 128, fin + 192, dout, n_blocks, dw_partial, dbias_partial,
                                            stream, dh, fin, m12, dz);
}

extern "C" int p2r_stgcn_tconv_weight_grad_dz_amax(int N, int T, int V, int taps, const float *x, const float *fin,
                                                   const float *dout, const float *dh, const float *m12, float *dz,
                                                   int n_blocks, float *dw_partial, float *dbias_partial,
                                                   unsigned *amax_bits, void *stream) {
  if (N < 0 || T <= 0 || V != 53 || taps != 3 || n_blocks < 1 || !fin || !dh || !m12 || !dz || !amax_bits) return P2R_EINVAL;
  hipError_t e = hipMemsetAsync(amax_bits, 0, sizeof(unsigned), p2r_stream(stream));
  if (e != hipSuccess) return (int)e;
  if (N == 0) return P2R_OK;
  return tconv_dw_launch<3, 53, TW_F, true, true>(N, T, V, x, fin + 128, fin + 192, dout, n_blocks, dw_partial,
                                                  dbias_partial, stream, dh, fin, m12, dz, amax_bits);
}
```

Measured before the change: 804.3 samples/s.

## Use buffer loads with OOB handling, split rows, unroll wgrad, tune tconv tiles

Replaces global loads in the pointwise GEMM, wgrad, SA and gather-grad kernels with AMDGPU buffer resource loads, so out-of-range reads come back as zero instead of needing explicit branches. Partial column tiles are now supported so L need not be a multiple of 64. A row-split parameter spreads pointwise GEMM work across more blocks. The wgrad kernel is templated on an unroll factor with dynamic LDS. Launch bounds are raised to two blocks per CU, and a smaller-tile tconv variant covers the V=20 case. Adds size guards for the 2 GB buffer limit and risks register pressure from the larger unrolled state.

```diff
diff --git a/pose2room_amd/csrc/p2r_common.h b/pose2room_amd/csrc/p2r_common.h
--- a/pose2room_amd/csrc/p2r_common.h
+++ b/pose2room_amd/csrc/p2r_common.h
@@ -55,6 +55,21 @@
   return dx * dx + dy * dy + dz * dz;
 }
 
+typedef __amdgpu_buffer_rsrc_t p2r_buf_t;
+#define P2R_BUF_MAX 0x7fffffffLL
+#define P2R_BUF_OOB 0x80000000u
+__device__ __forceinline__ p2r_buf_t p2r_buf(const void *base, unsigned bytes) {
+  return __builtin_amdgcn_make_buffer_rsrc(const_cast<void *>(base), 0, (int)bytes, 0x00020000);
+}
+__device__ __forceinline__ float p2r_buf_f32(p2r_buf_t d, unsigned off) {
+  return __uint_as_float(__builtin_amdgcn_raw_buffer_load_b32(d, (int)off, 0, 0));
+}
+__device__ __forceinline__ float4 p2r_buf_f32x4(p2r_buf_t d, unsigned off) {
+  typedef unsigned p2r_u32x4 __attribute__((ext_vector_type(4)));
+  const p2r_u32x4 u = __builtin_amdgcn_raw_buffer_load_b128(d, (int)off, 0, 0);
+  return make_float4(__uint_as_float(u.x), __uint_as_float(u.y), __uint_as_float(u.z), __uint_as_float(u.w));
+}
+
 __device__ __forceinline__ float p2r_row16_sum(float v) {
   v += __int_as_float(__builtin_amdgcn_update_dpp(0, __float_as_int(v), 0xB1, 0xf, 0xf, false));
   v += __int_as_float(__builtin_amdgcn_update_dpp(0, __float_as_int(v), 0x4E, 0xf, 0xf, false));
diff --git a/pose2room_amd/csrc/pw_layers.hip b/pose2room_amd/csrc/pw_layers.hip
--- a/pose2room_amd/csrc/pw_layers.hip
+++ b/pose2room_amd/csrc/pw_layers.hip
@@ -7,79 +7,105 @@
 
 struct PwJobs { p2r_pw_job j[P2R_PW_MAX_JOBS]; };
 
-__global__ __launch_bounds__(256) void pw_gemm_kernel(PwJobs jobs, int L, int colblocks) {
+__global__ __launch_bounds__(256, 2) void pw_gemm_kernel(PwJobs jobs, int L, int tiles_l, int colblocks, int rsplit) {
   extern __shared__ float tile[];
-  const p2r_pw_job &J = jobs.j[blockIdx.x / colblocks];
+  const int jp = blockIdx.x / colblocks;
+  const p2r_pw_job &J = jobs.j[jp / rsplit];
+  const int part = jp % rsplit;
   const int cb = blockIdx.x % colblocks;
-  const int col0 = cb * PW_COLS;
-  const int b = col0 / L, l0 = col0 - b * L;
-  const int tid = threadIdx.x, lane = tid & 63, wave = tid >> 6;
+  const int b = __builtin_amdgcn_readfirstlane(cb / tiles_l), l0 = (cb - b * tiles_l) * PW_COLS;
+  const int ncols = min(PW_COLS, L - l0);
+  const int tid = threadIdx.x, lane = tid & 63, wave = __builtin_amdgcn_readfirstlane(tid >> 6);
   const int g = lane >> 4, r = lane & 15;
   const int K = J.k, kpad = (K + 15) & ~15, rows = J.rows;
 
   if (!J.x_nlc) {
     const int c4 = tid & 15;
-    const size_t base = (size_t)b * J.x_ctot * L + l0 + 4 * c4;
+    const unsigned slab = 4u * (unsigned)K * (unsigned)L;
+    const p2r_buf_t dx = p2r_buf(J.x + (size_t)b * J.x_ctot * L, slab);
+    const p2r_buf_t dz = p2r_buf((J.tr_mode == 2 ? J.x2 : J.x) + (size_t)b * J.x_ctot * L, slab);
+    const int nv = ncols - 4 * c4;
+    const bool vec = (L & 3) == 0;
     for (int row = tid >> 4; row < kpad; row += 16) {
-      float4 v = make_float4(0.f, 0.f, 0.f, 0.f);
-      if (row < K) {
-        v = *reinterpret_cast<const float4 *>(J.x + base + (size_t)row * L);
-        if (J.tr_mode == 1) {
-          const float s = J.tr[row], t = J.tr[J.tr_ld + row];
-          v.x = fmaxf(v.x * s + t, 0.f); v.y = fmaxf(v.y * s + t, 0.f);
-          v.z = fmaxf(v.z * s + t, 0.f); v.w = fmaxf(v.w * s + t, 0.f);
-        } else if (J.tr_mode == 2) {
-          const float4 z = *reinterpret_cast<const float4 *>(J.x2 + base + (size_t)row * L);
-          const float a = J.tr[row], bq = J.tr[J.tr_ld + row], c = J.tr[2 * J.tr_ld + row];
-          v.x = a * v.x + bq * z.x + c; v.y = a * v.y + bq * z.y + c;
-          v.z = a * v.z + bq * z.z + c; v.w = a * v.w + bq * z.w + c;
-        }
-      }
+      const unsigned off = 4u * ((unsigned)row * (unsigned)L + (unsigned)(l0 + 4 * c4));
+      const int rc = min(row, K - 1);
+      float4 v, z = make_float4(0.f, 0.f, 0.f, 0.f);
+      if (vec) {
+        v = p2r_buf_f32x4(dx, off);
+        if (J.tr_mode == 2) z = p2r_buf_f32x4(dz, off);
+      } else {
+        v = make_float4(p2r_buf_f32(dx, off), p2r_buf_f32(dx, off + 4), p2r_buf_f32(dx, off + 8), p2r_buf_f32(dx, off + 12));
+        if (J.tr_mode == 2)
+          z = make_float4(p2r_buf_f32(dz, off), p2r_buf_f32(dz, off + 4), p2r_buf_f32(dz, off + 8), p2r_buf_f32(dz, off + 12));
+      }
+      if (J.tr_mode == 1) {
+        const float s = J.tr[rc], t = J.tr[J.tr_ld + rc];
+        v.x = fmaxf(v.x * s + t, 0.f); v.y = fmaxf(v.y * s + t, 0.f);
+        v.z = fmaxf(v.z * s + t, 0.f); v.w = fmaxf(v.w * s + t, 0.f);
+      } else if (J.tr_mode == 2) {
+        const float a = J.tr[rc], bq = J.tr[J.tr_ld + rc], c = J.tr[2 * J.tr_ld + rc];
+        v.x = a * v.x + bq * z.x + c; v.y = a * v.y + bq * z.y + c;
+        v.z = a * v.z + bq * z.z + c; v.w = a * v.w + bq * z.w + c;
+      }
+      const bool rok = row < K;
+      v.x = rok && nv > 0 ? v.x : 0.f; v.y = rok && nv > 1 ? v.y : 0.f;
+      v.z = rok && nv > 2 ? v.z : 0.f; v.w = rok && nv > 3 ? v.w : 0.f;
       *reinterpret_cast<float4 *>(tile + row * PW_RS + 4 * c4) = v;
-    }
-  } else if ((K & 3) != 0 || (J.x_ctot & 3) != 0) {
-    const int col = tid & 63;
-    const size_t base = ((size_t)b * L + l0 + col) * J.x_ctot;
-    for (int row = tid >> 6; row < kpad; row += 4) {
-      float v = 0.f;
-      if (row < K) {
-        v = J.x[base + row];
-        if (J.tr_mode == 1) v = fmaxf(v * J.tr[row] + J.tr[J.tr_ld + row], 0.f);
-        else if (J.tr_mode == 2) v = J.tr[row] * v + J.tr[J.tr_ld + row] * J.x2[base + row] + J.tr[2 * J.tr_ld + row];
-      }
-      tile[row * PW_RS + col] = v;
     }
   } else {
     const int col = tid & 63;
-    const size_t base = ((size_t)b * L + l0 + col) * J.x_ctot;
-    for (int c4 = tid >> 6; c4 < (kpad >> 2); c4 += 4) {
-      const int row = 4 * c4;
-      float v[4] = {0.f, 0.f, 0.f, 0.f};
-      if (row < K) {
-        const float4 u = *reinterpret_cast<const float4 *>(J.x + base + row);
-        v[0] = u.x; v[1] = u.y; v[2] = u.z; v[3] = u.w;
-        if (J.tr_mode == 1) {
-#pragma unroll
-          for (int e = 0; e < 4; ++e) v[e] = fmaxf(v[e] * J.tr[row + e] + J.tr[J.tr_ld + row + e], 0.f);
-        } else if (J.tr_mode == 2) {
-          const float4 z4 = *reinterpret_cast<const float4 *>(J.x2 + base + row);
-          const float z[4] = {z4.x, z4.y, z4.z, z4.w};
-#pragma unroll
-          for (int e = 0; e < 4; ++e)
-            v[e] = J.tr[row + e] * v[e] + J.tr[J.tr_ld + row + e] * z[e] + J.tr[2 * J.tr_ld + row + e];
+    const bool cok = col < ncols;
+    const unsigned slab = 4u * ((unsigned)(L - 1) * (unsigned)J.x_ctot + (unsigned)K);
+    const p2r_buf_t dx = p2r_buf(J.x + (size_t)b * L * J.x_ctot, slab);
+    const p2r_buf_t dz = p2r_buf((J.tr_mode == 2 ? J.x2 : J.x) + (size_t)b * L * J.x_ctot, slab);
+    const unsigned base = 4u * (unsigned)(l0 + col) * (unsigned)J.x_ctot;
+    if ((K & 3) != 0 || (J.x_ctot & 3) != 0) {
+      for (int row = wave; row < kpad; row += 4) {
+        float v = 0.f;
+        if (row < K) {
+          v = p2r_buf_f32(dx, base + 4u * row);
+          if (J.tr_mode == 1) v = fmaxf(v * J.tr[row] + J.tr[J.tr_ld + row], 0.f);
+          else if (J.tr_mode == 2)
+            v = J.tr[row] * v + J.tr[J.tr_ld + row] * p2r_buf_f32(dz, base + 4u * row) + J.tr[2 * J.tr_ld + row];
         }
-      }
-#pragma unroll
-      for (int e = 0; e < 4; ++e) tile[(row + e) * PW_RS + col] = v[e];
+        tile[row * PW_RS + col] = cok ? v : 0.f;
+      }
+    } else {
+      for (int c4 = wave; c4 < (kpad >> 2); c4 += 4) {
+        const int row = 4 * c4;
+        float v[4] = {0.f, 0.f, 0.f, 0.f};
+        if (row < K) {
+          const float4 u = p2r_buf_f32x4(dx, base + 4u * row);
+          v[0] = u.x; v[1] = u.y; v[2] = u.z; v[3] = u.w;
+          if (J.tr_mode == 1) {
+#pragma unroll
+            for (int e = 0; e < 4; ++e) v[e] = fmaxf(v[e] * J.tr[row + e] + J.tr[J.tr_ld + row + e], 0.f);
+          } else if (J.tr_mode == 2) {
+            const float4 z4 = p2r_buf_f32x4(dz, base + 4u * row);
+            const float z[4] = {z4.x, z4.y, z4.z, z4.w};
+#pragma unroll
+            for (int e = 0; e < 4; ++e)
+              v[e] = J.tr[row + e] * v[e] + J.tr[J.tr_ld + row + e] * z[e] + J.tr[2 * J.tr_ld + row + e];
+          }
+        }
+#pragma unroll
+        for (int e = 0; e < 4; ++e) tile[(row + e) * PW_RS + col] = cok ? v[e] : 0.f;
+      }
     }
   }
   __syncthreads();
 
   const int mtiles = (rows + 15) >> 4;
-  const int per = (mtiles + 3) >> 2;
-  const int lo = wave * per, hi = min(lo + per, mtiles);
+  const int mper = (mtiles + rsplit - 1) / rsplit;
+  const int m_lo = part * mper, m_hi = min(m_lo + mper, mtiles);
+  const int per = (max(m_hi - m_lo, 0) + 3) >> 2;
+  const int lo = m_lo + wave * per, hi = min(lo + per, m_hi);
   const int nch = kpad >> 4;
   const bool nlc_vec = J.out_nlc && (rows & 3) == 0 && (J.out_ctot & 3) == 0 && (((size_t)J.out) & 15) == 0;
+  bool cv[4];
+#pragma unroll
+  for (int n = 0; n < 4; ++n) cv[n] = 16 * n + r < ncols;
+  const float inv_cols = 1.f / (float)ncols;
   for (int mt0 = lo; mt0 < hi; mt0 += 4) {
     const int nmt = min(4, hi - mt0);
     floatx4v acc[4][4];
@@ -102,34 +128,36 @@
       for (int q = 0; q < 4; ++q) {
         const int row = row0 + q;
         const bool ok = row < rows;
+        const int rc = min(row, rows - 1);
         if (J.epilogue == 0) {
-          const float bb = (J.bias && ok) ? J.bias[row] : 0.f;
+          const float bb = J.bias ? J.bias[rc] : 0.f;
 #pragma unroll
           for (int n = 0; n < 4; ++n) v[q][n] = acc[m][n][q] + bb;
           if (J.stats) {
-            float s = (v[q][0] + v[q][1]) + (v[q][2] + v[q][3]);
+            float u[4];
+#pragma unroll
+            for (int n = 0; n < 4; ++n) u[n] = cv[n] ? v[q][n] : 0.f;
+            float s = (u[0] + u[1]) + (u[2] + u[3]);
             s = p2r_row16_sum(s);
-            const float mean = s * (1.f / 64.f);
+            const float mean = s * inv_cols;
             float d2 = 0.f;
 #pragma unroll
-            for (int n = 0; n < 4; ++n) { const float d = v[q][n] - mean; d2 += d * d; }
+            for (int n = 0; n < 4; ++n) { const float d = cv[n] ? v[q][n] - mean : 0.f; d2 += d * d; }
             d2 = p2r_row16_sum(d2);
             if (r == 0 && ok) {
               float *e = J.stats + ((size_t)cb * rows + row) * 3;
-              e[0] = 64.f; e[1] = mean; e[2] = d2;
+              e[0] = (float)ncols; e[1] = mean; e[2] = d2;
             }
           }
         } else {
-          float sc = 0.f, sh = 0.f, mean = 0.f, invstd = 0.f;
-          if (ok) {
-            mean = J.mfin[row]; invstd = J.mfin[J.mfin_ld + row];
-            sc = J.mfin[2 * J.mfin_ld + row]; sh = J.mfin[3 * J.mfin_ld + row];
-          }
+          const p2r_buf_t dmz = p2r_buf(J.mz + (size_t)b * J.mz_ctot * L, 4u * (unsigned)rows * (unsigned)L);
+          const float mean = J.mfin[rc], invstd = J.mfin[J.mfin_ld + rc];
+          const float sc = J.mfin[2 * J.mfin_ld + rc], sh = J.mfin[3 * J.mfin_ld + rc];
           float s1 = 0.f, s2 = 0.f;
 #pragma unroll
           for (int n = 0; n < 4; ++n) {
-            float z = 0.f;
-            if (ok) z = J.mz[((size_t)b * J.mz_ctot + row) * L + l0 + 16 * n + r];
+            const unsigned off = 4u * ((unsigned)row * (unsigned)L + (unsigned)(l0 + 16 * n + r));
+            const float z = p2r_buf_f32(dmz, cv[n] ? off : P2R_BUF_OOB);
             const float gv = (z * sc + sh > 0.f) ? acc[m][n][q] : 0.f;
             v[q][n] = gv;
             s1 += gv;
@@ -151,11 +179,13 @@
           if (row0 + q < rows) {
             float *o = J.out + ((size_t)b * J.out_ctot + row0 + q) * L + l0 + r;
 #pragma unroll
-            for (int n = 0; n < 4; ++n) o[16 * n] = v[q][n];
+            for (int n = 0; n < 4; ++n)
+              if (cv[n]) o[16 * n] = v[q][n];
           }
       } else {
 #pragma unroll
         for (int n = 0; n < 4; ++n) {
+          if (!cv[n]) continue;
           float *o = J.out + ((size_t)b * L + l0 + 16 * n + r) * J.out_ctot + row0;
           if (nlc_vec) {
             if (row0 < rows) *reinterpret_cast<float4 *>(o) = make_float4(v[0][n], v[1][n], v[2][n], v[3][n]);
@@ -171,33 +201,39 @@
 }
 
 struct PwWJobs { p2r_pw_wjob j[P2R_PW_MAX_JOBS]; int blk0[P2R_PW_MAX_JOBS + 1]; };
-constexpr int PWW_RS = 68;
-
-__device__ __forceinline__ void pww_fetch(const float *__restrict__ p, int ctot, int nlc, int L, int b, int l0, int row_lo,
-                                          int nrows, int tid, float4 (&v)[4]) {
+__device__ __forceinline__ void pww_fetch(p2r_buf_t d, int ctot, int nlc, int L, int l0, int row_lo, int nrows, int tid,
+                                          float4 (&v)[4]) {
 #pragma unroll
   for (int i = 0; i < 4; ++i) {
-    v[i] = make_float4(0.f, 0.f, 0.f, 0.f);
     if (!nlc) {
-      const int row = row_lo + (tid >> 4) + 16 * i;
-      if (row < nrows) v[i] = *reinterpret_cast<const float4 *>(p + ((size_t)b * ctot + row) * L + l0 + 4 * (tid & 15));
+      const unsigned off = 4u * ((unsigned)(row_lo + (tid >> 4) + 16 * i) * (unsigned)L + (unsigned)(l0 + 4 * (tid & 15)));
+      if ((L & 3) == 0) v[i] = p2r_buf_f32x4(d, off);
+      else v[i] = make_float4(p2r_buf_f32(d, off), p2r_buf_f32(d, off + 4), p2r_buf_f32(d, off + 8), p2r_buf_f32(d, off + 12));
     } else {
       const int row = row_lo + 4 * ((tid >> 6) + 4 * i);
-      const float *q = p + ((size_t)b * L + l0 + (tid & 63)) * ctot;
+      const unsigned off = 4u * ((unsigned)(l0 + (tid & 63)) * (unsigned)ctot + (unsigned)row);
       if (((nrows | ctot) & 3) == 0) {
-        if (row < nrows) v[i] = *reinterpret_cast<const float4 *>(q + row);
+        v[i] = p2r_buf_f32x4(d, row < nrows ? off : P2R_BUF_OOB);
       } else {
-        if (row + 0 < nrows) v[i].x = q[row + 0];
-        if (row + 1 < nrows) v[i].y = q[row + 1];
-        if (row + 2 < nrows) v[i].z = q[row + 2];
-        if (row + 3 < nrows) v[i].w = q[row + 3];
-      }
-    }
-  }
-}
-
-__global__ __launch_bounds__(256) void pw_wgrad_kernel(PwWJobs jobs, int L, int chunks) {
-  __shared__ float as[64 * PWW_RS], bs[64 * PWW_RS];
+        v[i].x = p2r_buf_f32(d, row + 0 < nrows ? off + 0 : P2R_BUF_OOB);
+        v[i].y = p2r_buf_f32(d, row + 1 < nrows ? off + 4 : P2R_BUF_OOB);
+        v[i].z = p2r_buf_f32(d, row + 2 < nrows ? off + 8 : P2R_BUF_OOB);
+        v[i].w = p2r_buf_f32(d, row + 3 < nrows ? off + 12 : P2R_BUF_OOB);
+      }
+    }
+  }
+}
+
+__device__ __forceinline__ p2r_buf_t pww_slab(const float *p, int ctot, int nlc, int L, int b, int nrows) {
+  return nlc ? p2r_buf(p + (size_t)b * L * ctot, 4u * ((unsigned)(L - 1) * (unsigned)ctot + (unsigned)nrows))
+             : p2r_buf(p + (size_t)b * ctot * L, 4u * (unsigned)nrows * (unsigned)L);
+}
+
+template <int U>
+__global__ __launch_bounds__(256, 2) void pw_wgrad_kernel(PwWJobs jobs, int L, int tiles_l, int chunks) {
+  constexpr int RS = 64 * U + 4;
+  extern __shared__ float wg_lds[];
+  float *as = wg_lds, *bs = wg_lds + 64 * RS;
   int ji = 0;
 #pragma unroll
   for (int i = 1; i < P2R_PW_MAX_JOBS; ++i)
@@ -210,7 +246,7 @@
   const int tm = t / tiles_n, tn = t % tiles_n;
   const int cps = (chunks + J.split - 1) / J.split;
   const int c_lo = sp * cps, c_hi = min(c_lo + cps, chunks);
-  const int tid = threadIdx.x, lane = tid & 63, wave = tid >> 6;
+  const int tid = threadIdx.x, lane = tid & 63, wave = __builtin_amdgcn_readfirstlane(tid >> 6);
   const int g = lane >> 4, r = lane & 15;
   const int row_a = 64 * tm, row_b = 64 * tn;
 
@@ -220,89 +256,102 @@
   float bsum = 0.f;
   const bool want_b = J.db_part != nullptr && tn == 0;
 
-  float4 ra[4], ra2[4], rb[4];
-#pragma unroll
-  for (int i = 0; i < 4; ++i) ra2[i] = make_float4(0.f, 0.f, 0.f, 0.f);
-  if (c_lo < c_hi) {
-    const int col0 = c_lo * 64, b = col0 / L, l0 = col0 - b * L;
-    pww_fetch(J.x, J.x_ctot, J.x_nlc, L, b, l0, row_a, rows, tid, ra);
-    if (J.tr_mode == 2) pww_fetch(J.x2, J.x_ctot, J.x_nlc, L, b, l0, row_a, rows, tid, ra2);
-    pww_fetch(J.y, J.y_ctot, J.y_nlc, L, b, l0, row_b, K, tid, rb);
-  }
-  for (int c = c_lo; c < c_hi; ++c) {
+  float4 ra[U][4], ra2[U][4], rb[U][4];
+  int ncol[U];
+#pragma unroll
+  for (int h = 0; h < U; ++h)
+#pragma unroll
+    for (int i = 0; i < 4; ++i) ra[h][i] = ra2[h][i] = rb[h][i] = make_float4(0.f, 0.f, 0.f, 0.f);
+  auto fetch = [&](int c0) __attribute__((always_inline)) {
+#pragma unroll
+    for (int h = 0; h < U; ++h) {
+      ncol[h] = 0;
+      if (c0 + h < c_hi) {
+        const int b = __builtin_amdgcn_readfirstlane((c0 + h) / tiles_l), l0 = (c0 + h - b * tiles_l) * 64;
+        ncol[h] = min(64, L - l0);
+        pww_fetch(pww_slab(J.x, J.x_ctot, J.x_nlc, L, b, rows), J.x_ctot, J.x_nlc, L, l0, row_a, rows, tid, ra[h]);
+        if (J.tr_mode == 2)
+          pww_fetch(pww_slab(J.x2, J.x_ctot, J.x_nlc, L, b, rows), J.x_ctot, J.x_nlc, L, l0, row_a, rows, tid, ra2[h]);
+        pww_fetch(pww_slab(J.y, J.y_ctot, J.y_nlc, L, b, K), J.y_ctot, J.y_nlc, L, l0, row_b, K, tid, rb[h]);
+      }
+    }
+  };
+  fetch(c_lo);
+  for (int c = c_lo; c < c_hi; c += U) {
     __syncthreads();
 #pragma unroll
-    for (int i = 0; i < 4; ++i) {
-      const float va[4] = {ra[i].x, ra[i].y, ra[i].z, ra[i].w};
-      const float vz[4] = {ra2[i].x, ra2[i].y, ra2[i].z, ra2[i].w};
-      const float vb[4] = {rb[i].x, rb[i].y, rb[i].z, rb[i].w};
-      if (!J.x_nlc) {
-        const int lr = (tid >> 4) + 16 * i, row = row_a + lr;
-        float o[4] = {0.f, 0.f, 0.f, 0.f};
-        if (row < rows) {
+    for (int h = 0; h < U; ++h) {
+      const int nv = ncol[h] - 4 * (tid & 15);
+      const bool cok = (tid & 63) < ncol[h];
+#pragma unroll
+      for (int i = 0; i < 4; ++i) {
+        const float va[4] = {ra[h][i].x, ra[h][i].y, ra[h][i].z, ra[h][i].w};
+        const float vz[4] = {ra2[h][i].x, ra2[h][i].y, ra2[h][i].z, ra2[h][i].w};
+        const float vb[4] = {rb[h][i].x, rb[h][i].y, rb[h][i].z, rb[h][i].w};
+        if (!J.x_nlc) {
+          const int lr = (tid >> 4) + 16 * i, row = row_a + lr, rc = min(row, rows - 1);
+          float o[4];
           if (J.tr_mode == 2) {
-            const float a = J.tr[row], bq = J.tr[J.tr_ld + row], cc = J.tr[2 * J.tr_ld + row];
+            const float a = J.tr[rc], bq = J.tr[J.tr_ld + rc], cc = J.tr[2 * J.tr_ld + rc];
 #pragma unroll
             for (int e = 0; e < 4; ++e) o[e] = a * va[e] + bq * vz[e] + cc;
           } else {
 #pragma unroll
             for (int e = 0; e < 4; ++e) o[e] = va[e];
           }
+#pragma unroll
+          for (int e = 0; e < 4; ++e) o[e] = row < rows && e < nv ? o[e] : 0.f;
+          *reinterpret_cast<float4 *>(as + lr * RS + 64 * h + 4 * (tid & 15)) = make_float4(o[0], o[1], o[2], o[3]);
+        } else {
+#pragma unroll
+          for (int e = 0; e < 4; ++e) {
+            const int lr = 4 * ((tid >> 6) + 4 * i) + e, row = row_a + lr, rc = min(row, rows - 1);
+            const float v = J.tr_mode == 2 ? J.tr[rc] * va[e] + J.tr[J.tr_ld + rc] * vz[e] + J.tr[2 * J.tr_ld + rc] : va[e];
+            as[lr * RS + 64 * h + (tid & 63)] = row < rows && cok ? v : 0.f;
+          }
         }
-        *reinterpret_cast<float4 *>(as + lr * PWW_RS + 4 * (tid & 15)) = make_float4(o[0], o[1], o[2], o[3]);
-      } else {
-#pragma unroll
-        for (int e = 0; e < 4; ++e) {
-          const int lr = 4 * ((tid >> 6) + 4 * i) + e, row = row_a + lr;
-          float v = 0.f;
-          if (row < rows) v = J.tr_mode == 2 ? J.tr[row] * va[e] + J.tr[J.tr_ld + row] * vz[e] + J.tr[2 * J.tr_ld + row] : va[e];
-          as[lr * PWW_RS + (tid & 63)] = v;
-        }
-      }
-      if (!J.y_nlc) {
-        const int lr = (tid >> 4) + 16 * i, row = row_b + lr;
-        float o[4] = {0.f, 0.f, 0.f, 0.f};
-        if (row < K) {
+        if (!J.y_nlc) {
+          const int lr = (tid >> 4) + 16 * i, row = row_b + lr, rc = min(row, K - 1);
+          float o[4];
           if (J.ytr) {
-            const float sc = J.ytr[row], sh = J.ytr[J.ytr_ld + row];
+            const float sc = J.ytr[rc], sh = J.ytr[J.ytr_ld + rc];
 #pragma unroll
             for (int e = 0; e < 4; ++e) o[e] = fmaxf(vb[e] * sc + sh, 0.f);
           } else {
 #pragma unroll
             for (int e = 0; e < 4; ++e) o[e] = vb[e];
           }
+#pragma unroll
+          for (int e = 0; e < 4; ++e) o[e] = row < K && e < nv ? o[e] : 0.f;
+          *reinterpret_cast<float4 *>(bs + lr * RS + 64 * h + 4 * (tid & 15)) = make_float4(o[0], o[1], o[2], o[3]);
+        } else {
+#pragma unroll
+          for (int e = 0; e < 4; ++e) {
+            const int lr = 4 * ((tid >> 6) + 4 * i) + e, row = row_b + lr, rc = min(row, K - 1);
+            const float v = J.ytr ? fmaxf(vb[e] * J.ytr[rc] + J.ytr[J.ytr_ld + rc], 0.f) : vb[e];
+            bs[lr * RS + 64 * h + (tid & 63)] = row < K && cok ? v : 0.f;
+          }
         }
-        *reinterpret_cast<float4 *>(bs + lr * PWW_RS + 4 * (tid & 15)) = make_float4(o[0], o[1], o[2], o[3]);
-      } else {
-#pragma unroll
-        for (int e = 0; e < 4; ++e) {
-          const int lr = 4 * ((tid >> 6) + 4 * i) + e, row = row_b + lr;
-          float v = 0.f;
-          if (row < K) v = J.ytr ? fmaxf(vb[e] * J.ytr[row] + J.ytr[J.ytr_ld + row], 0.f) : vb[e];
-          bs[lr * PWW_RS + (tid & 63)] = v;
-        }
       }
     }
     __syncthreads();
-    if (c + 1 < c_hi) {
-      const int col0 = (c + 1) * 64, b = col0 / L, l0 = col0 - b * L;
-      pww_fetch(J.x, J.x_ctot, J.x_nlc, L, b, l0, row_a, rows, tid, ra);
-      if (J.tr_mode == 2) pww_fetch(J.x2, J.x_ctot, J.x_nlc, L, b, l0, row_a, rows, tid, ra2);
-      pww_fetch(J.y, J.y_ctot, J.y_nlc, L, b, l0, row_b, K, tid, rb);
-    }
+    fetch(c + U);
 #pragma unroll 4
-    for (int k = 0; k < 64; k += 4) {
-      const float bv = bs[(16 * wave + r) * PWW_RS + k + g];
+    for (int k = 0; k < 64 * U; k += 4) {
+      const float bv = bs[(16 * wave + r) * RS + k + g];
 #pragma unroll
       for (int mt = 0; mt < 4; ++mt)
-        acc[mt] = __builtin_amdgcn_mfma_f32_16x16x4f32(as[(16 * mt + r) * PWW_RS + k + g], bv, acc[mt], 0, 0, 0);
+        acc[mt] = __builtin_amdgcn_mfma_f32_16x16x4f32(as[(16 * mt + r) * RS + k + g], bv, acc[mt], 0, 0, 0);
     }
     if (want_b) {
-      const float *rowp = as + (tid >> 2) * PWW_RS + 16 * (tid & 3);
-      float s = 0.f;
-#pragma unroll
-      for (int i = 0; i < 16; ++i) s += rowp[i];
-      bsum += s;
+#pragma unroll
+      for (int h = 0; h < U; ++h) {
+        const float *rowp = as + (tid >> 2) * RS + 64 * h + 16 * (tid & 3);
+        float s = 0.f;
+#pragma unroll
+        for (int i = 0; i < 16; ++i) s += rowp[i];
+        bsum += s;
+      }
     }
   }
   float *outp = J.dw_part + (size_t)sp * rows * K;
@@ -536,11 +585,14 @@
 
 }
 
+constexpr int PW_SPLIT_WGS = 256;
+
 extern "C" int p2r_pw_gemm(int njobs, const p2r_pw_job *jobs, int B, int L, void *stream) {
-  if (njobs < 1 || njobs > P2R_PW_MAX_JOBS || B < 0 || L <= 0 || L % PW_COLS != 0 || !jobs) return P2R_EINVAL;
+  if (njobs < 1 || njobs > P2R_PW_MAX_JOBS || B < 0 || L <= 0 || !jobs) return P2R_EINVAL;
   if (B == 0) return P2R_OK;
   PwJobs pj;
-  int kmax = 0;
+  int kmax = 0, rmax = 0;
+  const long long Lp = (long long)L + PW_COLS;
   for (int i = 0; i < njobs; ++i) {
     const p2r_pw_job &j = jobs[i];
     const int kpad = (j.k + 15) & ~15;
@@ -550,25 +602,33 @@
     if (j.tr_mode != 0 && !j.tr) return P2R_EINVAL;
     if (j.epilogue == 1 && (!j.mz || !j.mfin)) return P2R_EINVAL;
     if (j.epilogue != 0 && j.epilogue != 1) return P2R_EINVAL;
+    if (4 * (j.x_nlc ? Lp * j.x_ctot + kpad : (kpad + 1) * Lp) > P2R_BUF_MAX) return P2R_EINVAL;
+    if (j.epilogue == 1 && 4 * ((long long)j.rows + 16) * Lp > P2R_BUF_MAX) return P2R_EINVAL;
     pj.j[i] = j;
     if (kpad > kmax) kmax = kpad;
-  }
-  const int colblocks = (int)((long long)B * L / PW_COLS);
+    if (j.rows > rmax) rmax = j.rows;
+  }
+  const int tiles_l = p2r_cdiv(L, PW_COLS);
+  const long long cbl = (long long)B * tiles_l;
+  if (cbl * njobs * 2 > 0x7fffffffLL) return P2R_EINVAL;
+  const int colblocks = (int)cbl;
+  const int rsplit = (cbl * njobs <= PW_SPLIT_WGS && rmax >= 128) ? 2 : 1;
   const int lds = kmax * PW_RS * (int)sizeof(float);
   static unsigned char lds_ok[P2R_MAX_DEVICES];
   hipError_t e = p2r_allow_big_lds(pw_gemm_kernel, lds_ok, PW_KMAX * PW_RS * (int)sizeof(float));
   if (e != hipSuccess) return (int)e;
-  hipLaunchKernelGGL(pw_gemm_kernel, dim3((unsigned)(njobs * colblocks)), dim3(256), lds, p2r_stream(stream), pj, L,
-                     colblocks);
+  hipLaunchKernelGGL(pw_gemm_kernel, dim3((unsigned)(njobs * rsplit * colblocks)), dim3(256), lds, p2r_stream(stream), pj,
+                     L, tiles_l, colblocks, rsplit);
   P2R_LAUNCH_CHECK();
   return P2R_OK;
 }
 
 extern "C" int p2r_pw_wgrad(int njobs, const p2r_pw_wjob *jobs, int B, int L, void *stream) {
-  if (njobs < 1 || njobs > P2R_PW_MAX_JOBS || B < 0 || L <= 0 || L % 64 != 0 || !jobs) return P2R_EINVAL;
+  if (njobs < 1 || njobs > P2R_PW_MAX_JOBS || B < 0 || L <= 0 || !jobs) return P2R_EINVAL;
   if (B == 0) return P2R_OK;
   PwWJobs pj;
-  int total = 0;
+  int total = 0, smax = 1;
+  const long long Lp = (long long)L + 64;
   for (int i = 0; i < P2R_PW_MAX_JOBS + 1; ++i) pj.blk0[i] = 0x7fffffff;
   for (int i = 0; i < njobs; ++i) {
     const p2r_pw_wjob &j = jobs[i];
@@ -576,13 +636,28 @@
     if (j.tr_mode != 0 && j.tr_mode != 2) return P2R_EINVAL;
     if (j.tr_mode == 2 && (!j.x2 || !j.tr)) return P2R_EINVAL;
     if ((((size_t)j.x) & 15) != 0 || (((size_t)j.y) & 15) != 0 || (j.x2 && (((size_t)j.x2) & 15) != 0)) return P2R_EINVAL;
+    if (4 * (j.x_nlc ? Lp * j.x_ctot + j.rows + 64 : ((long long)j.rows + 64) * Lp) > P2R_BUF_MAX) return P2R_EINVAL;
+    if (4 * (j.y_nlc ? Lp * j.y_ctot + j.k + 64 : ((long long)j.k + 64) * Lp) > P2R_BUF_MAX) return P2R_EINVAL;
     pj.j[i] = j;
     pj.blk0[i] = total;
     total += ((j.rows + 63) / 64) * ((j.k + 63) / 64) * j.split;
+    if (j.split > smax) smax = j.split;
   }
   pj.blk0[0] = 0;
-  const int chunks = (int)((long long)B * L / 64);
-  hipLaunchKernelGGL(pw_wgrad_kernel, dim3((unsigned)total), dim3(256), 0, p2r_stream(stream), pj, L, chunks);
+  const int tiles_l = p2r_cdiv(L, 64);
+  const long long ch = (long long)B * tiles_l;
+  if (ch > 0x7fffffffLL) return P2R_EINVAL;
+  const int chunks = (int)ch;
+  if (chunks / smax >= 4) {
+    constexpr int lds = 2 * 64 * (64 * 2 + 4) * (int)sizeof(float);
+    static unsigned char lds_ok[P2R_MAX_DEVICES];
+    hipError_t e = p2r_allow_big_lds(pw_wgrad_kernel<2>, lds_ok, lds);
+    if (e != hipSuccess) return (int)e;
+    hipLaunchKernelGGL(pw_wgrad_kernel<2>, dim3((unsigned)total), dim3(256), lds, p2r_stream(stream), pj, L, tiles_l, chunks);
+  } else {
+    constexpr int lds = 2 * 64 * (64 + 4) * (int)sizeof(float);
+    hipLaunchKernelGGL(pw_wgrad_kernel<1>, dim3((unsigned)total), dim3(256), lds, p2r_stream(stream), pj, L, tiles_l, chunks);
+  }
   P2R_LAUNCH_CHECK();
   return P2R_OK;
 }
diff --git a/pose2room_amd/csrc/sa_votes.hip b/pose2room_amd/csrc/sa_votes.hip
--- a/pose2room_amd/csrc/sa_votes.hip
+++ b/pose2room_amd/csrc/sa_votes.hip
@@ -34,10 +34,10 @@
   float *hs = lds;
   __shared__ int s_idx[SA_BALLS][SA_S];
 
-  const int tid = threadIdx.x, lane = tid & 63, wave = tid >> 6;
+  const int tid = threadIdx.x, lane = tid & 63, wave = __builtin_amdgcn_readfirstlane(tid >> 6);
   const int g = lane >> 4, r = lane & 15;
   const int groups = (m + SA_BALLS - 1) / SA_BALLS;
-  const int batch = blockIdx.x / groups;
+  const int batch = __builtin_amdgcn_readfirstlane(blockIdx.x / groups);
   const int j0 = (blockIdx.x % groups) * SA_BALLS;
   const float *pts = xyz + (size_t)batch * n * 3;
   const float *feat = features + (size_t)batch * SA_C * n;
@@ -50,10 +50,11 @@
       const float cy = new_xyz[((size_t)batch * m + j) * 3 + 1];
       const float cz = new_xyz[((size_t)batch * m + j) * 3 + 2];
       const unsigned long long lt_mask = (lane == 0) ? 0ull : (~0ull >> (64 - lane));
+      const p2r_buf_t dp = p2r_buf(pts, 12u * (unsigned)n);
       for (int k0 = 0; k0 < n && cnt < SA_S; k0 += 64) {
         const int k = k0 + lane;
-        bool hit = false;
-        if (k < n) hit = p2r_sqdist(cx, cy, cz, pts[k * 3 + 0], pts[k * 3 + 1], pts[k * 3 + 2]) < radius2;
+        const float px = p2r_buf_f32(dp, 12u * k), py = p2r_buf_f32(dp, 12u * k + 4), pz = p2r_buf_f32(dp, 12u * k + 8);
+        const bool hit = (p2r_sqdist(cx, cy, cz, px, py, pz) < radius2) & (k < n);
         const unsigned long long mask = __ballot(hit);
         if (mask != 0ull) {
           if (cnt == 0) first = k0 + (int)__builtin_ctzll(mask);
@@ -76,7 +77,7 @@
     const int col = tid & 63;
     const int src = s_idx[col >> 4][col & 15];
     const int jc = j0 + (col >> 4);
-    for (int c = tid >> 6; c < SA_C; c += 4) {
+    for (int c = wave; c < SA_C; c += 4) {
       const float v = feat[(size_t)c * n + src];
       gs[c * SA_RS + col] = v;
       if (TRAIN && jc < m) G[(((size_t)batch * SA_C + c) * m + jc) * SA_S + (col & 15)] = v;
@@ -116,7 +117,9 @@
         for (int off = 8; off >= 1; off >>= 1) {
           const float ov = __shfl_xor(v, off, 16);
           const int oa = __shfl_xor(am, off, 16);
-          if (ov > v || (ov == v && oa < am)) { v = ov; am = oa; }
+          const bool take = (ov > v) | ((ov == v) & (oa < am));
+          v = take ? ov : v;
+          am = take ? oa : am;
         }
         const int j = j0 + nt;
         if (r == 0 && j < m) {
@@ -138,22 +141,24 @@
   extern __shared__ float lds[];
   float *zs = lds;
   float *ys = lds;
-  const int tid = threadIdx.x, lane = tid & 63, wave = tid >> 6;
+  const int tid = threadIdx.x, lane = tid & 63, wave = __builtin_amdgcn_readfirstlane(tid >> 6);
   const int g = lane >> 4, r = lane & 15;
   const int groups = (m + SA_BALLS - 1) / SA_BALLS;
-  const int batch = blockIdx.x / groups;
+  const int batch = __builtin_amdgcn_readfirstlane(blockIdx.x / groups);
   const int j0 = (blockIdx.x % groups) * SA_BALLS;
 
   {
     const int col = tid & 63, ball = col >> 4, smp = col & 15;
     const int j = j0 + ball;
-    for (int c = tid >> 6; c < SA_C; c += 4) {
-      float v = 0.f;
-      if (j < m) {
-        const size_t o = ((size_t)batch * SA_C + c) * m + j;
-        if ((int)amax[o] == smp && out[o] > 0.f) v = dout[o];
-        dZ2[o * SA_S + smp] = v;
-      }
+    const size_t slab = (size_t)batch * SA_C * m;
+    const unsigned cm = (unsigned)SA_C * (unsigned)m;
+    const p2r_buf_t da = p2r_buf(amax + slab, cm), dq = p2r_buf(out + slab, 4u * cm), dd = p2r_buf(dout + slab, 4u * cm);
+    for (int c = wave; c < SA_C; c += 4) {
+      const unsigned e = (unsigned)c * (unsigned)m + (unsigned)j;
+      const int am = (int)__builtin_amdgcn_raw_buffer_load_b8(da, (int)(j < m ? e : P2R_BUF_OOB), 0, 0);
+      const float po = p2r_buf_f32(dq, j < m ? 4u * e : P2R_BUF_OOB), dv = p2r_buf_f32(dd, j < m ? 4u * e : P2R_BUF_OOB);
+      const float v = ((am == smp) & (po > 0.f)) ? dv : 0.f;
+      if (j < m) dZ2[(slab + e) * SA_S + smp] = v;
       zs[c * SA_RS + col] = v;
     }
   }
@@ -258,6 +263,7 @@
   if (train && (!H || !amax)) return P2R_EINVAL;
   if (nsample != SA_S || C0 != SA_C || C1 != SA_C || C2 != SA_C) return P2R_EINVAL;
   if (b == 0 || m == 0) return P2R_OK;
+  if (12LL * ((long long)n + 64) > P2R_BUF_MAX) return P2R_EINVAL;
   const int groups = (m + SA_BALLS - 1) / SA_BALLS;
   const size_t lds = (size_t)SA_C * SA_RS * sizeof(float);
   auto kern = train ? sa_votes_kernel<true> : sa_votes_kernel<false>;
@@ -275,6 +281,7 @@
                                      float *dZ2, float *dZ1, float *dG, void *stream) {
   if (b < 0 || m < 0 || nsample != SA_S || C != SA_C) return P2R_EINVAL;
   if (b == 0 || m == 0) return P2R_OK;
+  if (4LL * SA_C * ((long long)m + SA_BALLS) > P2R_BUF_MAX) return P2R_EINVAL;
   const int groups = (m + SA_BALLS - 1) / SA_BALLS;
   const size_t lds = (size_t)SA_C * SA_RS * sizeof(float);
   static unsigned char lds_ok[P2R_MAX_DEVICES];
diff --git a/pose2room_amd/csrc/seed_ops.hip b/pose2room_amd/csrc/seed_ops.hip
--- a/pose2room_amd/csrc/seed_ops.hip
+++ b/pose2room_amd/csrc/seed_ops.hip
@@ -29,15 +29,19 @@
   __shared__ int hits[GF_TT][GF_MAXHIT];
   __shared__ int nhit[GF_TT];
   const int chunks = (T + GF_TT - 1) / GF_TT;
-  const int b = blockIdx.x / chunks, t0 = (blockIdx.x - b * chunks) * GF_TT;
-  const int tid = threadIdx.x, lane = tid & 63, wave = tid >> 6;
+  const int b = __builtin_amdgcn_readfirstlane(blockIdx.x / chunks), t0 = (blockIdx.x - b * chunks) * GF_TT;
+  const int tid = threadIdx.x, lane = tid & 63, wave = __builtin_amdgcn_readfirstlane(tid >> 6);
+  const p2r_buf_t di = p2r_buf(inds + (size_t)b * S, 8u * (unsigned)S);
+  const p2r_buf_t dd = p2r_buf(dout + (size_t)b * S * C * J, 4u * (unsigned)S * (unsigned)(C * J));
   for (int f = 2 * wave; f < 2 * wave + 2; ++f) {
     const long long t = t0 + f;
     int cnt = 0;
     const unsigned long long lt = lane == 0 ? 0ull : (~0ull >> (64 - lane));
     for (int s0 = 0; s0 < S; s0 += 64) {
       const int s = s0 + lane;
-      const bool hit = s < S && inds[(size_t)b * S + s] == t;
+      typedef unsigned gf_u32x2 __attribute__((ext_vector_type(2)));
+      const gf_u32x2 w = __builtin_amdgcn_raw_buffer_load_b64(di, 8 * s, 0, 0);
+      const bool hit = (s < S) & ((long long)(((unsigned long long)w.y << 32) | w.x) == t);
       const unsigned long long m = __ballot(hit);
       const int slot = cnt + (int)__builtin_popcountll(m & lt);
       if (hit && slot < GF_MAXHIT) hits[f][slot] = s;
@@ -53,23 +57,22 @@
     const int cnt = nhit[f];
     float *xb = dx + ((size_t)b * C * T + t0) * J + e;
     if (cnt <= 2) {
-      const float *r0 = dout + ((size_t)b * S + (cnt > 0 ? hits[f][0] : 0)) * n + j;
-      const float *r1 = dout + ((size_t)b * S + (cnt > 1 ? hits[f][1] : 0)) * n + j;
+      const unsigned r0 = cnt > 0 ? 4u * ((unsigned)hits[f][0] * (unsigned)n + (unsigned)j) : P2R_BUF_OOB;
+      const unsigned r1 = cnt > 1 ? 4u * ((unsigned)hits[f][1] * (unsigned)n + (unsigned)j) : P2R_BUF_OOB;
       int c = 0;
       for (; c + 8 <= C; c += 8) {
         float v[8];
 #pragma unroll
         for (int u = 0; u < 8; ++u) {
-          v[u] = cnt > 0 ? r0[(c + u) * J] : 0.f;
-          if (cnt > 1) v[u] += r1[(c + u) * J];
+          const float v0 = p2r_buf_f32(dd, r0 + 4u * (unsigned)((c + u) * J)), v1 = p2r_buf_f32(dd, r1 + 4u * (unsigned)((c + u) * J));
+          v[u] = cnt > 1 ? v0 + v1 : v0;
         }
 #pragma unroll
         for (int u = 0; u < 8; ++u) xb[(size_t)(c + u) * T * J] = v[u];
       }
       for (; c < C; ++c) {
-        float v = cnt > 0 ? r0[c * J] : 0.f;
-        if (cnt > 1) v += r1[c * J];
-        xb[(size_t)c * T * J] = v;
+        const float v0 = p2r_buf_f32(dd, r0 + 4u * (unsigned)(c * J)), v1 = p2r_buf_f32(dd, r1 + 4u * (unsigned)(c * J));
+        xb[(size_t)c * T * J] = cnt > 1 ? v0 + v1 : v0;
       }
       continue;
     }
@@ -214,6 +217,7 @@
                                       float *dx, void *stream) {
   if (b < 0 || c <= 0 || t <= 0 || j <= 0 || s < 0) return P2R_EINVAL;
   if (b == 0) return P2R_OK;
+  if (4LL * ((long long)s + 64) * c * j > P2R_BUF_MAX || 8LL * ((long long)s + 64) > P2R_BUF_MAX) return P2R_EINVAL;
   hipLaunchKernelGGL(gather_frames_grad_kernel, dim3((unsigned)(b * ((t + GF_TT - 1) / GF_TT))), dim3(256), 0,
                      p2r_stream(stream), c, t, j, s, dout, inds, dx);
   P2R_LAUNCH_CHECK();
diff --git a/pose2room_amd/csrc/stgcn_tconv.hip b/pose2room_amd/csrc/stgcn_tconv.hip
--- a/pose2room_amd/csrc/stgcn_tconv.hip
+++ b/pose2room_amd/csrc/stgcn_tconv.hip
@@ -7,16 +7,17 @@
 constexpr int TC_C = 64;
 constexpr int TC_NPO = 384;
 constexpr int TC_THREADS = 512;
-constexpr int TC_NT = 3;
-
-template <int TAPS>
+constexpr int TC_PE_V = 20;
+
+template <int TAPS, int NPO = TC_NPO>
 __global__ __launch_bounds__(TC_THREADS, 2) void tconv_fused_kernel(
     int n_seq, int T, int V, int F, int tiles_per_seq, int row_len, const float *__restrict__ x,
     const float *__restrict__ scale, const float *__restrict__ shift, const float *__restrict__ W,
     const float *__restrict__ bias, float *__restrict__ out, float *__restrict__ stats_partial) {
   extern __shared__ float hs[];
   constexpr int HALO = (TAPS - 1) / 2;
-  constexpr int NCH = TAPS == 1 ? TC_NPO / 64 : 8;
+  constexpr int NT = NPO / (16 * (TC_THREADS / 64));
+  constexpr int NCH = TAPS == 1 ? NPO / 64 : 8;
 
   const int tid = threadIdx.x, lane = tid & 63, wave = __builtin_amdgcn_readfirstlane(tid >> 6);
   const int g = lane >> 4, r = lane & 15;
@@ -76,23 +77,23 @@
     __syncthreads();
     if (tile + (int)gridDim.x < total_tiles) issue_loads(tile + gridDim.x);
 
-    int colv[TC_NT], base[TC_NT];
-    bool valid[TC_NT];
-#pragma unroll
-    for (int i = 0; i < TC_NT; ++i) {
-      const int col = (wave * TC_NT + i) * 16 + r;
+    int colv[NT], base[NT];
+    bool valid[NT];
+#pragma unroll
+    for (int i = 0; i < NT; ++i) {
+      const int col = (wave * NT + i) * 16 + r;
       colv[i] = col;
       valid[i] = col < ncols;
       base[i] = valid[i] ? col : 0;
     }
-    floatx4c acc[TC_NT][4];
+    floatx4c acc[NT][4];
 #pragma unroll
     for (int m = 0; m < 4; ++m)
 #pragma unroll
       for (int q = 0; q < 4; ++q) {
         const float bv = bias ? bias[16 * m + 4 * g + q] : 0.f;
 #pragma unroll
-        for (int i = 0; i < TC_NT; ++i) acc[i][m][q] = bv;
+        for (int i = 0; i < NT; ++i) acc[i][m][q] = bv;
       }
 
     const float *hg = hs + g * 16 * row_len;
@@ -110,7 +111,7 @@
         }
       }
 #pragma unroll
-      for (int i = 0; i < TC_NT; ++i) {
+      for (int i = 0; i < NT; ++i) {
         const float *hb = hg + base[i] + p * V + 8 * hf * row_len;
         float b[8];
 #pragma unroll
@@ -130,7 +131,7 @@
         const int row = 16 * m + 4 * g + q;
         float s1 = 0.f, s2 = 0.f;
 #pragma unroll
-        for (int i = 0; i < TC_NT; ++i) {
+        for (int i = 0; i < NT; ++i) {
           if (!valid[i]) continue;
           const float v = acc[i][m][q];
           og[(size_t)row * row_stride + colv[i]] = v;
@@ -390,7 +391,9 @@
                                 const float *W, const float *bias, float *out, float *stats_partial,
                                 int *n_partials, void *stream) {
   constexpr int HALO = (TAPS - 1) / 2;
-  int F = TC_NPO / V;
+  constexpr int NPO_PE = 256;
+  const bool pe = TAPS == 1 && V == TC_PE_V && (long long)N * p2r_cdiv(T, NPO_PE / V) <= 256;
+  int F = (pe ? NPO_PE : TC_NPO) / V;
   if (F < 1) return P2R_EINVAL;
   if (F > T) F = T;
   const int tiles_per_seq = p2r_cdiv(T, F);
@@ -399,16 +402,21 @@
   const size_t lds = (size_t)TC_C * row_len * sizeof(float) + (size_t)(TC_THREADS / 64) * 2 * TC_C * sizeof(float);
   if (lds > 160 * 1024 || row_len > 512) return P2R_EINVAL;
   if ((long long)T * V >= (1LL << 29)) return P2R_EINVAL;
-  static unsigned char lds_ok[P2R_MAX_DEVICES];
-  {
-    hipError_t e = p2r_allow_big_lds(tconv_fused_kernel<TAPS>, lds_ok);
-    if (e != hipSuccess) return (int)e;
-  }
   const long long tiles = (long long)N * tiles_per_seq;
   if (tiles > 0x7fffffffLL) return P2R_EINVAL;
   const int blocks = (int)(tiles < 256 ? tiles : 256);
   if (n_partials) *n_partials = blocks;
   if (!out) return P2R_OK;
+  if constexpr (TAPS == 1) {
+    if (pe)
+      return p2r_launch_big_lds<tconv_fused_kernel<1, NPO_PE>>(blocks, TC_THREADS, lds, stream, N, T, V, F, tiles_per_seq,
+                                                               row_len, x, scale, shift, W, bias, out, stats_partial);
+  }
+  static unsigned char lds_ok[P2R_MAX_DEVICES];
+  {
+    hipError_t e = p2r_allow_big_lds(tconv_fused_kernel<TAPS>, lds_ok);
+    if (e != hipSuccess) return (int)e;
+  }
   hipLaunchKernelGGL(tconv_fused_kernel<TAPS>, dim3(blocks), dim3(TC_THREADS), lds, p2r_stream(stream), N, T, V,
                      F, tiles_per_seq, row_len, x, scale, shift, W, bias, out, stats_partial);
   P2R_LAUNCH_CHECK();
```

Result: no change. 808.6 samples/s, median of 6 (+0.5%).
